# pixeli99/SVD_Xtend

Measured on NVIDIA H100. Metric: SVD UNet train-step frames/sec @ 14x320x512 bf16, higher is better.
Workload: dtype bf16

## Files before the change

### svd_xtend_b200/csrc/tapgemm.cu

```cuda
#include "tapgemm_common.cuh"

namespace svdx {

template <int BN, int TA, int TB>
__device__ __forceinline__ void tile_mainloop(int kb0, int kb1, uint32_t sA, uint32_t sB, uint32_t bar_full, uint32_t bar_empty,
                                           uint32_t sAcc, int wg, int& stage, uint32_t& phase) {
  float acc[BN / 2];
#pragma unroll
  for (int i = 0; i < BN / 2; ++i) acc[i] = 0.f;
  const int lane = threadIdx.x & 31;
  const uint32_t astep = TA ? (2048 >> 4) : (32 >> 4), bstep = TB ? (2048 >> 4) : (32 >> 4);
  int prev_stage = -1;
  for (int kb = kb0; kb < kb1; ++kb) {
    mbar_wait_mma(bar_full + 8 * stage, phase);
    const uint32_t aaddr = sA + stage * A_STAGE_BYTES + wg * 8192;
    const uint32_t baddr = sB + stage * B_STAGE_BYTES;
    const uint64_t ad0 = make_smem_desc_sw128(aaddr, 8192, 1024);
    const uint64_t bd0 = make_smem_desc_sw128(baddr, 8192, 1024);
    wgmma_fence();
#pragma unroll
    for (int j = 0; j < BLOCK_K / 16; ++j) {
      const uint32_t accumulate = (kb > kb0 || j > 0) ? 1u : 0u;
      if constexpr (BN == 32) wgmma_ss_n32<TA, TB>(acc, ad0 + j * astep, bd0 + j * bstep, accumulate);
      else if constexpr (BN == 64) wgmma_ss_n64<TA, TB>(acc, ad0 + j * astep, bd0 + j * bstep, accumulate);
      else if constexpr (BN == 96) wgmma_ss_n96<TA, TB>(acc, ad0 + j * astep, bd0 + j * bstep, accumulate);
      else if constexpr (BN == 128) wgmma_ss_n128<TA, TB>(acc, ad0 + j * astep, bd0 + j * bstep, accumulate);
      else wgmma_ss_n160<TA, TB>(acc, ad0 + j * astep, bd0 + j * bstep, accumulate);
    }
    wgmma_commit();
    wgmma_wait<1>();
    reg_fence(acc);
    if (prev_stage >= 0) {
      __syncwarp();
      if (lane == 0) mbar_arrive(bar_empty + 8 * prev_stage);
    }
    prev_stage = stage;
    if (++stage == STAGES) { stage = 0; phase ^= 1; }
  }
  wgmma_wait<0>();
  reg_fence(acc);
  __syncwarp();
  if (lane == 0 && prev_stage >= 0) mbar_arrive(bar_empty + 8 * prev_stage);

  const int r0 = wg * 64 + ((threadIdx.x >> 5) & 3) * 16 + (lane >> 2);
  const uint32_t base = sAcc + (uint32_t)(r0 * ACC_LD + 2 * (lane & 3)) * 4u;
#pragma unroll
  for (int j = 0; j < BN / 8; ++j) {
#pragma unroll
    for (int h = 0; h < 2; ++h)
      asm volatile("st.shared.v2.f32 [%0], {%1, %2};" ::"r"(base + (uint32_t)(h * 8 * ACC_LD + 8 * j) * 4u), "f"(acc[4 * j + 2 * h]),
                   "f"(acc[4 * j + 2 * h + 1]) : "memory");
  }
}

template <int TA, int TB>
SVDX_DEVINL void tile_mainloop_bn(int bn, int kb0, int kb1, uint32_t sA, uint32_t sB, uint32_t bar_full, uint32_t bar_empty, uint32_t sAcc,
                                  int wg, int& stage, uint32_t& phase) {
  switch (bn) {
    case 32: tile_mainloop<32, TA, TB>(kb0, kb1, sA, sB, bar_full, bar_empty, sAcc, wg, stage, phase); break;
    case 64: tile_mainloop<64, TA, TB>(kb0, kb1, sA, sB, bar_full, bar_empty, sAcc, wg, stage, phase); break;
    case 96: tile_mainloop<96, TA, TB>(kb0, kb1, sA, sB, bar_full, bar_empty, sAcc, wg, stage, phase); break;
    case 128: tile_mainloop<128, TA, TB>(kb0, kb1, sA, sB, bar_full, bar_empty, sAcc, wg, stage, phase); break;
    default: tile_mainloop<160, TA, TB>(kb0, kb1, sA, sB, bar_full, bar_empty, sAcc, wg, stage, phase); break;
  }
}

template <int EPI>
__global__ void __launch_bounds__(NUM_THREADS, 1) tapgemm_kernel(const __grid_constant__ TapGemmKParams p) {
  extern __shared__ uint8_t smem_raw[];
  const uint32_t smem_base = (smem_u32(smem_raw) + 1023u) & ~1023u;
  const uint32_t sA = smem_base;
  const uint32_t sB = smem_base + STAGES * A_STAGE_BYTES;
  const uint32_t sAcc = sB + STAGES * B_STAGE_BYTES;
  const uint32_t sEpi = sAcc + ACC_BYTES;
  const uint32_t sBar = sEpi + NUM_EPI_WARPS * EPI_STAGE_BYTES;
  const uint32_t bar_full = sBar;
  const uint32_t bar_empty = sBar + 8 * STAGES;

  const int warp = threadIdx.x >> 5;
  const int lane = threadIdx.x & 31;

  if (warp == PRODUCER_WARP && lane == 0) {
    prefetch_tmap(&p.tma);
    prefetch_tmap(&p.tmb);
    for (int i = 0; i < STAGES; ++i) {
      mbar_init(bar_full + 8 * i, 1);
      mbar_init(bar_empty + 8 * i, NUM_EPI_WARPS);
    }
    fence_barrier_init();
  }
  __syncthreads();

  const int total_tiles = p.m_tiles * p.n_tiles * p.split_k;
  const int b_bytes = p.block_n * BLOCK_K * 2;

  if (warp == PRODUCER_WARP) {
    const bool conv_par = (p.a_mode == SVDX_A_CONV2D) && !p.a_mn && !p.b_mn && !p.geglu && !p.wtiles && !p.im2col && (BLOCK_M / p.W) <= 32;
    if (conv_par) {
      int stage = 0;
      uint32_t phase = 0;
      for (int tile = blockIdx.x; tile < total_tiles; tile += gridDim.x) {
        const int nt = tile % p.n_tiles;
        const int mt = (tile / p.n_tiles) % p.m_tiles;
        const int ks = tile / (p.n_tiles * p.m_tiles);
        const int kb0 = ks * p.kb_per_split;
        const int kb1 = min(kb0 + p.kb_per_split, p.kb_total);
        const int n0 = nt * p.block_n;
        ConvBox bx;
        conv_tile_boxes(p, mt, lane, bx);
        const CUtensorMap* amap = bx.lg == 0 ? &p.tma : &p.tma_bh[bx.lg - 1];
        int tap = kb0 / p.kb_per_tap;
        int kci = kb0 - tap * p.kb_per_tap;
        for (int kb = kb0; kb < kb1; ++kb) {
          const uint32_t full = bar_full + 8 * stage;
          if (lane == 0) {
            mbar_wait_mma(bar_empty + 8 * stage, phase ^ 1);
            mbar_expect_tx(full, A_STAGE_BYTES + b_bytes);
          }
          __syncwarp();
          const int kc = kci * BLOCK_K;
          if (bx.active)
            tma_load_4d(amap, full, sA + stage * A_STAGE_BYTES + bx.dst_off, kc, p.tap_d0[tap], bx.hh + p.tap_d1[tap],
                        bx.nvalid ? bx.n + p.tap_d2[tap] : (1 << 28));
          if (lane == 0) tma_load_2d(&p.tmb, full, sB + stage * B_STAGE_BYTES, tap * p.K + kc, n0);
          if (++kci == p.kb_per_tap) { kci = 0; ++tap; }
          if (++stage == STAGES) { stage = 0; phase ^= 1; }
        }
      }
    } else if (p.a_mn && p.b_mn && p.b_mode != 1) {
      int stage = 0;
      uint32_t phase = 0;
      const int nb = p.block_n / 64;
      for (int tile = blockIdx.x; tile < total_tiles; tile += gridDim.x) {
        const int nt = tile % p.n_tiles;
        const int mt = (tile / p.n_tiles) % p.m_tiles;
        const int ks = tile / (p.n_tiles * p.m_tiles);
        const int kb0 = ks * p.kb_per_split;
        const int kb1 = min(kb0 + p.kb_per_split, p.kb_total);
        const int n0 = nt * p.block_n;
        int g = 0, kbi = kb0;
        if (p.b_mode == 2) { g = kb0 / p.kb_per_group; kbi = kb0 - g * p.kb_per_group; }
        const int shift = p.b_mode == 2 ? p.tap_d0[0] : 0;
        for (int kb = kb0; kb < kb1; ++kb) {
          const uint32_t full = bar_full + 8 * stage;
          if (lane == 0) {
            mbar_wait_mma(bar_empty + 8 * stage, phase ^ 1);
            mbar_expect_tx(full, A_STAGE_BYTES + b_bytes);
          }
          __syncwarp();
          const uint32_t dA = sA + stage * A_STAGE_BYTES;
          const uint32_t dB = sB + stage * B_STAGE_BYTES;
          if (p.b_mode == 2) {
            const int k0 = kbi * BLOCK_K;
            if (lane < 2) tma_load_3d(&p.tma, full, dA + lane * 8192, mt * BLOCK_M + 64 * lane, k0, g);
            else if (lane < 2 + nb) tma_load_3d(&p.tmb, full, dB + (lane - 2) * 8192, n0 + 64 * (lane - 2), k0 + shift, g);
            if (++kbi == p.kb_per_group) { kbi = 0; ++g; }
          } else {
            if (lane < 2) tma_load_2d(&p.tma, full, dA + lane * 8192, mt * BLOCK_M + 64 * lane, kb * BLOCK_K);
            else if (lane < 2 + nb) tma_load_2d(&p.tmb, full, dB + (lane - 2) * 8192, n0 + 64 * (lane - 2), kb * BLOCK_K);
          }
          if (++stage == STAGES) { stage = 0; phase ^= 1; }
        }
      }
    } else if (lane == 0) {
      int stage = 0;
      uint32_t phase = 0;
      for (int tile = blockIdx.x; tile < total_tiles; tile += gridDim.x) {
        const int nt = tile % p.n_tiles;
        const int mt = (tile / p.n_tiles) % p.m_tiles;
        const int ks = tile / (p.n_tiles * p.m_tiles);
        const int kb0 = ks * p.kb_per_split;
        const int kb1 = min(kb0 + p.kb_per_split, p.kb_total);
        const int n0 = nt * (p.geglu ? p.block_n / 2 : p.block_n);
        int iw = 0, ih = 0, in = 0;
        if (p.im2col && p.a_mode == SVDX_A_CONV2D) {
          const int row = mt * BLOCK_M / p.W;
          iw = mt * BLOCK_M - row * p.W;
          in = row / p.H;
          ih = row - in * p.H;
        }
        int tap = kb0 / p.kb_per_tap;
        int kci = kb0 - tap * p.kb_per_tap - 1;
        for (int kb = kb0; kb < kb1; ++kb) {
          if (++kci == p.kb_per_tap) { kci = 0; ++tap; }
          mbar_wait_mma(bar_empty + 8 * stage, phase ^ 1);
          const uint32_t full = bar_full + 8 * stage;
          mbar_expect_tx(full, A_STAGE_BYTES + b_bytes);
          const uint32_t dA = sA + stage * A_STAGE_BYTES;
          const uint32_t dB = sB + stage * B_STAGE_BYTES;
          const int kc = kci * BLOCK_K;
          if (p.a_mn) {
            if (p.b_mode == 2) {
              const int g = kb / p.kb_per_group;
              const int k0 = (kb - g * p.kb_per_group) * BLOCK_K;
              tma_load_3d(&p.tma, full, dA, mt * BLOCK_M, k0, g);
              tma_load_3d(&p.tma, full, dA + 8192, mt * BLOCK_M + 64, k0, g);
            } else {
              tma_load_2d(&p.tma, full, dA, mt * BLOCK_M, kb * BLOCK_K);
              tma_load_2d(&p.tma, full, dA + 8192, mt * BLOCK_M + 64, kb * BLOCK_K);
            }
          } else if (p.a_mode == SVDX_A_ROWS) {
            const int g = mt / p.tiles_per_group;
            const int t = mt - g * p.tiles_per_group;
            tma_load_3d(&p.tma, full, dA, kc, t * BLOCK_M + p.tap_d0[tap], g);
          } else if (p.im2col) {
            tma_load_4d_im2col(&p.tma, full, dA, kc, iw - 1, ih - 1, in + p.tap_d2[tap], (uint16_t)(p.tap_d0[tap] + 1),
                               (uint16_t)(p.tap_d1[tap] + 1));
          } else if (p.wtiles) {
            const int row = mt / p.wtiles;
            const int w0 = (mt - row * p.wtiles) * BLOCK_M;
            const int n = row / p.H;
            const int h = row - n * p.H;
            tma_load_4d(&p.tma, full, dA, kc, w0 + p.tap_d0[tap], h + p.tap_d1[tap], (n < p.nimg) ? n + p.tap_d2[tap] : (1 << 28));
          } else {
            const int R = BLOCK_M / p.W;
            const int dw = p.tap_d0[tap], dh = p.tap_d1[tap], dn = p.tap_d2[tap];
            int rowid = mt * R, left = R;
            uint32_t dst = dA;
            while (left > 0) {
              const int n = rowid / p.H;
              const int h = rowid - n * p.H;
              const int nn = (n < p.nimg) ? n + dn : (1 << 28);
              int run = min(left, p.H - h);
              int hh = h;
              while (run > 0) {
                int lg = min(p.max_bh_log2, 31 - __clz(run));
                const int bh = 1 << lg;
                tma_load_4d(lg == 0 ? &p.tma : &p.tma_bh[lg - 1], full, dst, kc, dw, hh + dh, nn);
                dst += bh * p.W * 128;
                hh += bh; run -= bh; left -= bh; rowid += bh;
              }
            }
          }
          if (p.b_mn && p.b_mode == 1 && p.im2col) {
            const int pix0 = kb * BLOCK_K;
            const int row = pix0 / p.W;
            const int n = row / p.H;
            for (int j = 0; j < p.block_n / 64; ++j)
              tma_load_4d_im2col(&p.tmb, full, dB + j * 8192, n0 + 64 * j, pix0 - row * p.W - 1, row - n * p.H - 1, n + p.tap_d2[0],
                                 (uint16_t)(p.tap_d0[0] + 1), (uint16_t)(p.tap_d1[0] + 1));
          } else if (p.b_mn && p.b_mode == 1) {
            const int dw = p.tap_d0[0], dh = p.tap_d1[0], dn = p.tap_d2[0];
            const int pix0 = kb * BLOCK_K;
            for (int j = 0; j < p.block_n / 64; ++j) {
              if (p.W >= 64) {
                const int row = pix0 / p.W;
                const int n = row / p.H;
                const int nn = (n < p.nimg) ? n + dn : (1 << 28);
                tma_load_4d(&p.tmb, full, dB + j * 8192, n0 + 64 * j, pix0 - row * p.W + dw, row - n * p.H + dh, nn);
              } else {
                const int R = 64 / p.W;
                for (int i = 0; i < R; ++i) {
                  const int row = pix0 / p.W + i;
                  const int n = row / p.H;
                  const int nn = (n < p.nimg) ? n + dn : (1 << 28);
                  tma_load_4d(&p.tmb, full, dB + j * 8192 + i * p.W * 128, n0 + 64 * j, dw, row - n * p.H + dh, nn);
                }
              }
            }
          } else if (p.b_mn && p.b_mode == 2) {
            const int g = kb / p.kb_per_group;
            const int k0 = (kb - g * p.kb_per_group) * BLOCK_K;
            for (int j = 0; j < p.block_n / 64; ++j)
              tma_load_3d(&p.tmb, full, dB + j * 8192, n0 + 64 * j, k0 + p.tap_d0[0], g);
          } else if (p.b_mn) {
            for (int j = 0; j < p.block_n / 64; ++j)
              tma_load_2d(&p.tmb, full, dB + j * 8192, n0 + 64 * j, kb * BLOCK_K);
          } else if (p.geglu) {
            const int h = p.block_n / 2;
            tma_load_2d(&p.tmb, full, dB, tap * p.K + kc, n0);
            tma_load_2d(&p.tmb, full, dB + h * 128, tap * p.K + kc, p.N / 2 + n0);
          } else {
            tma_load_2d(&p.tmb, full, dB, tap * p.K + kc, n0);
          }
          if (++stage == STAGES) { stage = 0; phase ^= 1; }
        }
      }
    }
  } else {
    const int wg = warp >> 2;
    const int q = warp & 3;
    const int half = warp >> 2;
    int stage = 0;
    uint32_t phase = 0;
    float s_acc = 1.f, s_r1 = 1.f, s_r2 = 1.f;
    if (p.scales) { s_acc = p.scales[0]; s_r1 = p.scales[1]; s_r2 = p.scales[2]; }
    const int n_out_total = p.geglu ? p.N / 2 : p.N;
    const int bn_out = p.geglu ? p.block_n / 2 : p.block_n;
    EpiStage st;
    st.base = sEpi + warp * EPI_STAGE_BYTES;
    st.off = 0;
    const uint32_t t_base = sAcc + (uint32_t)((q * 32 + lane) * ACC_LD) * 4u;
    for (int tile = blockIdx.x; tile < total_tiles; tile += gridDim.x) {
      const int nt = tile % p.n_tiles;
      const int mt = (tile / p.n_tiles) % p.m_tiles;
      const int ks = tile / (p.n_tiles * p.m_tiles);
      const int kb0 = ks * p.kb_per_split;
      const int kb1 = min(kb0 + p.kb_per_split, p.kb_total);
      const int n0 = nt * bn_out;
      long long m;
      bool row_ok;
      tile_row(p, mt, q * 32 + lane, m, row_ok);
      if (p.a_mode == SVDX_A_ROWS && !p.a_mn) {
        st.grp = mt / p.tiles_per_group;
        st.row0 = (mt - st.grp * p.tiles_per_group) * BLOCK_M + q * 32;
      } else {
        st.grp = 0;
        st.row0 = mt * BLOCK_M + q * 32;
      }
      long long m0;
      int valid_rows;
      if (p.a_mode == SVDX_A_ROWS && !p.a_mn) {
        m0 = (long long)st.grp * p.rows_per_group + st.row0;
        valid_rows = max(0, min(32, p.rows_per_group - st.row0));
      } else {
        m0 = st.row0;
        valid_rows = max(0, min(32, p.M - st.row0));
      }
      if constexpr (EPI == EPI_RES || EPI == EPI_RES_GN || EPI == EPI_FAST_GNB)
        prefetch_epilogue_operands(p, EPI, m0, valid_rows, n0, bn_out, n_out_total, lane, half);
      named_bar_sync(1, 32 * NUM_EPI_WARPS);
      if (p.a_mn && p.b_mn) tile_mainloop_bn<1, 1>(p.block_n, kb0, kb1, sA, sB, bar_full, bar_empty, sAcc, wg, stage, phase);
      else if (p.a_mn) tile_mainloop_bn<1, 0>(p.block_n, kb0, kb1, sA, sB, bar_full, bar_empty, sAcc, wg, stage, phase);
      else if (p.b_mn) tile_mainloop_bn<0, 1>(p.block_n, kb0, kb1, sA, sB, bar_full, bar_empty, sAcc, wg, stage, phase);
      else tile_mainloop_bn<0, 0>(p.block_n, kb0, kb1, sA, sB, bar_full, bar_empty, sAcc, wg, stage, phase);
      named_bar_sync(1, 32 * NUM_EPI_WARPS);
      if constexpr (EPI == EPI_FAST || EPI == EPI_FAST_GN) epilogue_fast<EPI == EPI_FAST_GN>(p, t_base, m, row_ok, n0, half, 0, bn_out, n_out_total, st.base, st.row0, st.grp, lane, m0, valid_rows);
      else if constexpr (EPI == EPI_FAST_IL || EPI == EPI_FAST_IL_GN) epilogue_fast<EPI == EPI_FAST_IL_GN, true>(p, t_base, m, row_ok, n0, half, 0, bn_out, n_out_total, st.base, st.row0, st.grp, lane, m0, valid_rows);
      else if constexpr (EPI == EPI_FAST_ACT) epilogue_fast<false, false, true>(p, t_base, m, row_ok, n0, half, 0, bn_out, n_out_total, st.base, st.row0, st.grp, lane, m0, valid_rows);
      else if constexpr (EPI == EPI_RES || EPI == EPI_RES_GN) epilogue_res<EPI == EPI_RES_GN>(p, t_base, m, row_ok, n0, half, 0, bn_out, n_out_total, s_acc, s_r1, s_r2, st.base, st.off, st.row0, st.grp, lane, m0, valid_rows);
      else if constexpr (EPI == EPI_GEGLU) epilogue_geglu(p, t_base, n0, half, bn_out, st.base, st.row0, st.grp, lane);
      else if constexpr (EPI == EPI_FAST_GNB) epilogue_fast_gnb(p, t_base, m, row_ok, n0, half, 0, bn_out, n_out_total, st.base, st.row0, st.grp, lane, m0, valid_rows);
      else epilogue_tile(p, t_base, m, row_ok, n0, half, bn_out, n_out_total, s_acc, s_r1, s_r2, st, lane);
    }
    if (lane == 0) bulk_wait<0>();
  }
}

}

using namespace svdx;

static int kernel_block_n(int block_n, bool step64) {
  const int step = step64 ? 64 : 32, cap = step64 ? 128 : MAX_BN;
  if (block_n <= cap) return block_n;
  for (int w = cap; w > step; w -= step)
    if (block_n % w == 0) return w;
  return step;
}

int svdx_tapgemm_fill(const SvdxTapGemm* d, TapGemmKParams& p) {
  if (!d || !d->a || !d->b || !d->out) return svdx_fail(SVDX_E_BADARG, "tapgemm: null pointer");
  const bool wide320 = d->block_n == 320;
  if (wide320 && (d->geglu || d->N % 320 || d->M < 512 || d->out_dtype != SVDX_OUT_BF16))
    return svdx_fail(SVDX_E_BADARG, "tapgemm: block_n 320 needs N %% 320 == 0, M >= 512 and a bf16 output without GEGLU");
  if (!wide320 && (d->block_n < 32 || d->block_n > 256 || d->block_n % 32))
    return svdx_fail(SVDX_E_BADARG, "tapgemm: block_n must be a multiple of 32 in [32,256] (or 320)");
  if (d->b_major_mn && d->block_n % 64) return svdx_fail(SVDX_E_BADARG, "tapgemm: block_n %% 64 for MN-major B");
  if (d->num_taps < 1 || d->num_taps > SVDX_MAX_TAPS) return svdx_fail(SVDX_E_BADARG, "tapgemm: num_taps");
  if (d->M <= 0 || d->N <= 0 || d->K <= 0) return svdx_fail(SVDX_E_BADARG, "tapgemm: empty problem");
  if (d->split_k < 1 || (d->split_k > 1 && d->out_dtype != SVDX_OUT_F32_ATOMIC)) return svdx_fail(SVDX_E_BADARG, "tapgemm: split_k needs atomic output");
  if (d->geglu && (d->N % 2 || d->block_n % 64 || d->b_major_mn || (d->N / 2) % (d->block_n / 2))) return svdx_fail(SVDX_E_BADARG, "tapgemm: geglu shape");
  if ((d->lda % 8) || (d->ldb % 8)) return svdx_fail(SVDX_E_BADARG, "tapgemm: lda/ldb must be multiples of 8 elements (16 B)");
  if ((reinterpret_cast<uintptr_t>(d->a) & 15) || (reinterpret_cast<uintptr_t>(d->b) & 15)) return svdx_fail(SVDX_E_BADARG, "tapgemm: operands must be 16 B aligned");
  if ((d->a_major_mn || d->b_major_mn) && (d->a_mode != SVDX_A_ROWS || d->num_taps != 1)) return svdx_fail(SVDX_E_BADARG, "tapgemm: MN-major operands only in single-tap ROWS mode");
  if (d->b_mode != 0 && !(d->a_major_mn && d->b_major_mn)) return svdx_fail(SVDX_E_BADARG, "tapgemm: b_mode needs MN-major A and B (weight-gradient form)");

  memset(&p, 0, sizeof(p));
  p.a_mode = d->a_mode; p.a_mn = d->a_major_mn; p.b_mn = d->b_major_mn;
  p.num_taps = d->num_taps;
  for (int i = 0; i < d->num_taps; ++i) { p.tap_d0[i] = d->tap_d0[i]; p.tap_d1[i] = d->tap_d1[i]; p.tap_d2[i] = d->tap_d2[i]; }
  const int block_n = kernel_block_n(d->block_n, d->b_major_mn || d->geglu);
  p.M = d->M; p.N = d->N; p.K = d->K; p.block_n = block_n; p.split_k = d->split_k;
  p.geglu = d->geglu;
  const int bn_out = d->geglu ? block_n / 2 : block_n;
  const int n_out = d->geglu ? d->N / 2 : d->N;
  p.n_tiles = (n_out + bn_out - 1) / bn_out;

  int rc;
  p.b_mode = d->b_mode;
  if (d->a_major_mn) {
    if (d->groups > 1 && d->b_mode != 2) return svdx_fail(SVDX_E_BADARG, "tapgemm: MN-major A requires groups==1");
    if (d->b_mode == 2) {
      uint64_t dims[3] = {(uint64_t)d->M, (uint64_t)d->rows_per_group, (uint64_t)d->groups};
      uint64_t strides[2] = {(uint64_t)d->lda * 2, (uint64_t)d->lda * 2 * (uint64_t)d->rows_per_group};
      uint32_t box[3] = {64, 64, 1};
      rc = svdx_make_tmap(&p.tma, d->a, 3, dims, strides, box);
    } else {
      uint64_t dims[2] = {(uint64_t)d->M, (uint64_t)d->K};
      uint64_t strides[1] = {(uint64_t)d->lda * 2};
      uint32_t box[2] = {64, 64};
      rc = svdx_make_tmap(&p.tma, d->a, 2, dims, strides, box);
    }
    p.rows_per_group = d->M; p.groups = 1; p.tiles_per_group = (d->M + BLOCK_M - 1) / BLOCK_M;
    p.m_tiles = p.tiles_per_group;
  } else if (d->a_mode == SVDX_A_ROWS) {
    if (d->rows_per_group <= 0 || d->groups <= 0 || (long long)d->rows_per_group * d->groups != d->M) return svdx_fail(SVDX_E_BADARG, "tapgemm: rows_per_group*groups != M");
    uint64_t dims[3] = {(uint64_t)d->K, (uint64_t)d->rows_per_group, (uint64_t)d->groups};
    uint64_t strides[2] = {(uint64_t)d->lda * 2, (uint64_t)d->lda * 2 * (uint64_t)d->rows_per_group};
    uint32_t box[3] = {64, 128, 1};
    rc = svdx_make_tmap(&p.tma, d->a, 3, dims, strides, box);
    p.rows_per_group = d->rows_per_group; p.groups = d->groups;
    p.tiles_per_group = (d->rows_per_group + BLOCK_M - 1) / BLOCK_M;
    p.m_tiles = p.tiles_per_group * d->groups;
  } else if (d->a_mode == SVDX_A_CONV2D) {
    const bool wide = d->W > 128;
    if (d->W <= 0 || d->H <= 0 || d->nimg <= 0) return svdx_fail(SVDX_E_BADARG, "tapgemm: conv2d needs W, H, images > 0");
    const bool boxes = wide ? (d->W % 128 == 0) : (128 % d->W == 0);
    uint64_t dims[4] = {(uint64_t)d->K, (uint64_t)d->W, (uint64_t)d->H, (uint64_t)d->nimg};
    uint64_t strides[3] = {(uint64_t)d->lda * 2, (uint64_t)d->lda * 2 * d->W, (uint64_t)d->lda * 2 * d->W * d->H};
    uint32_t box[4] = {64, (uint32_t)(wide ? 128 : d->W), 1, 1};
    p.max_bh_log2 = 0;
    if (!boxes) {
      for (int i = 0; i < d->num_taps; ++i)
        if (d->tap_d0[i] < -1 || d->tap_d0[i] > 1 || d->tap_d1[i] < -1 || d->tap_d1[i] > 1)
          return svdx_fail(SVDX_E_BADARG, "tapgemm: conv2d at a width with neither W | 128 nor 128 | W needs taps with |dw|, |dh| <= 1");
      rc = svdx_make_tmap_im2col(&p.tma, d->a, dims, strides, BLOCK_M);
      p.im2col = 1;
    } else {
      rc = svdx_make_tmap(&p.tma, d->a, 4, dims, strides, box);
    }
    p.wtiles = (wide && boxes) ? d->W / 128 : 0;
    for (int lg = 1; lg <= 4 && !rc && !wide && boxes; ++lg) {
      const int bh = 1 << lg;
      if (bh * d->W > BLOCK_M || bh > d->H) break;
      uint32_t boxh[4] = {64, (uint32_t)d->W, (uint32_t)bh, 1};
      rc = svdx_make_tmap(&p.tma_bh[lg - 1], d->a, 4, dims, strides, boxh);
      p.max_bh_log2 = lg;
    }
    p.W = d->W; p.H = d->H; p.nimg = d->M / (d->H * d->W);
    if ((long long)p.nimg * d->H * d->W != d->M) return svdx_fail(SVDX_E_BADARG, "tapgemm: conv2d M must be images*H*W");
    p.m_tiles = (d->M + BLOCK_M - 1) / BLOCK_M;
    p.rows_per_group = d->M; p.groups = 1; p.tiles_per_group = p.m_tiles;
  } else {
    return svdx_fail(SVDX_E_BADARG, "tapgemm: a_mode");
  }
  if (rc) return rc;

  if (d->b_major_mn && d->b_mode == 1) {
    if (d->W <= 0 || d->H <= 0 || d->nimg <= 0) return svdx_fail(SVDX_E_BADARG, "tapgemm: b_mode 1 needs W, H, images > 0");
    uint64_t dims[4] = {(uint64_t)d->N, (uint64_t)d->W, (uint64_t)d->H, (uint64_t)d->nimg};
    uint64_t strides[3] = {(uint64_t)d->ldb * 2, (uint64_t)d->ldb * 2 * d->W, (uint64_t)d->ldb * 2 * d->W * d->H};
    uint32_t box[4] = {64, (uint32_t)(d->W >= 64 ? 64 : d->W), 1, 1};
    if ((d->W < 64 && 64 % d->W) || (d->W >= 64 && d->W % 64)) {
      if (d->tap_d0[0] < -1 || d->tap_d0[0] > 1 || d->tap_d1[0] < -1 || d->tap_d1[0] > 1)
        return svdx_fail(SVDX_E_BADARG, "tapgemm: b_mode 1 at a width with neither W | 64 nor 64 | W needs a tap with |dw|, |dh| <= 1");
      rc = svdx_make_tmap_im2col(&p.tmb, d->b, dims, strides, 64);
      p.im2col = 1;
    } else {
      rc = svdx_make_tmap(&p.tmb, d->b, 4, dims, strides, box);
    }
    p.W = d->W; p.H = d->H; p.nimg = d->K / (d->W * d->H);
    if ((long long)p.nimg * d->W * d->H != d->K) return svdx_fail(SVDX_E_BADARG, "tapgemm: b_mode 1 K must be images*H*W");
  } else if (d->b_major_mn && d->b_mode == 2) {
    if (d->rows_per_group <= 0 || d->groups <= 0 || (long long)d->rows_per_group * d->groups != d->K) return svdx_fail(SVDX_E_BADARG, "tapgemm: b_mode 2 rows_per_group*groups != K");
    uint64_t dims[3] = {(uint64_t)d->N, (uint64_t)d->rows_per_group, (uint64_t)d->groups};
    uint64_t strides[2] = {(uint64_t)d->ldb * 2, (uint64_t)d->ldb * 2 * (uint64_t)d->rows_per_group};
    uint32_t box[3] = {64, 64, 1};
    rc = svdx_make_tmap(&p.tmb, d->b, 3, dims, strides, box);
    p.rows_per_group = d->rows_per_group; p.groups = d->groups;
  } else if (d->b_major_mn) {
    uint64_t dims[2] = {(uint64_t)d->N, (uint64_t)d->K};
    uint64_t strides[1] = {(uint64_t)d->ldb * 2};
    uint32_t box[2] = {64, 64};
    rc = svdx_make_tmap(&p.tmb, d->b, 2, dims, strides, box);
  } else {
    uint64_t dims[2] = {(uint64_t)d->K * d->num_taps, (uint64_t)d->N};
    uint64_t strides[1] = {(uint64_t)d->ldb * 2};
    uint32_t box[2] = {64, (uint32_t)(d->geglu ? block_n / 2 : block_n)};
    rc = svdx_make_tmap(&p.tmb, d->b, 2, dims, strides, box);
  }
  if (rc) return rc;

  p.kb_per_tap = (d->K + BLOCK_K - 1) / BLOCK_K;
  p.kb_total = p.kb_per_tap * d->num_taps;
  p.kb_per_group = p.kb_per_tap;
  if (d->b_mode == 2) {
    p.kb_per_group = (d->rows_per_group + BLOCK_K - 1) / BLOCK_K;
    p.kb_per_tap = p.kb_per_group * d->groups;
    p.kb_total = p.kb_per_tap;
  }
  p.kb_per_split = (p.kb_total + d->split_k - 1) / d->split_k;
  p.split_k = (p.kb_total + p.kb_per_split - 1) / p.kb_per_split;

  p.out = d->out; p.ldo = d->ldo; p.out_dtype = d->out_dtype;
  p.bias = d->bias; p.rowbias = d->rowbias; p.rowbias_div = d->rowbias_div > 0 ? d->rowbias_div : 1; p.ldrb = d->ldrb;
  p.res1 = reinterpret_cast<const bf16*>(d->res1); p.ldr1 = d->ldr1;
  p.res2 = reinterpret_cast<const bf16*>(d->res2); p.ldr2 = d->ldr2;
  p.scales = d->scales; p.pre = reinterpret_cast<bf16*>(d->pre); p.ldpre = d->ldpre;
  p.gn_sum = d->gn_sum; p.gn_ld = d->gn_ld; p.gn_rows = d->gn_rows;
  p.gnb_x = reinterpret_cast<const bf16*>(d->gnb_x); p.gnb_ldx = d->gnb_ldx; p.gnb_c1 = d->gnb_x2 ? d->gnb_c1 : d->N;
  p.gnb_x2 = reinterpret_cast<const bf16*>(d->gnb_x2); p.gnb_ldx2 = d->gnb_ldx2;
  p.gnb_ab = d->gnb_ab; p.gnb_sum = d->gnb_sum; p.gnb_rows = d->gnb_rows; p.gnb_silu = d->gnb_silu;
  {
    static int probe = -1;
    if (probe < 0) { const char* e = getenv("SVDX_EPI_PROBE"); probe = e ? atoi(e) : 0; }
    p.probe = probe;
  }
  {
    static int use = -1;
    if (use < 0) { const char* e = getenv("SVDX_TMA_STORE"); use = e ? atoi(e) : 1; }
    const bool grouped = (d->a_mode == SVDX_A_ROWS && !d->a_major_mn);
    const uint64_t R = grouped ? (uint64_t)d->rows_per_group : (uint64_t)d->M;
    const uint64_t G = grouped ? (uint64_t)d->groups : 1;
    const bool f32 = d->out_dtype != SVDX_OUT_BF16;
    const int esz = f32 ? 4 : 2;
    bool ok = use != 0 && (d->ldo * esz) % 16 == 0 && (reinterpret_cast<uintptr_t>(d->out) & 15) == 0;
    if (d->geglu && d->pre && ((d->N / 2) % 32 || (d->ldpre % 8) || (reinterpret_cast<uintptr_t>(d->pre) & 15))) ok = false;
    if (ok) {
      uint64_t dims[3] = {(uint64_t)n_out, R, G};
      uint64_t strides[2] = {(uint64_t)d->ldo * esz, (uint64_t)d->ldo * esz * R};
      uint32_t box[3] = {32, 32, 1};
      rc = svdx_make_tmap_ex(&p.tmo, d->out, f32, f32 ? 128 : 64, 3, dims, strides, box);
      if (rc) return rc;
      if (d->geglu && d->pre) {
        uint64_t pdims[3] = {(uint64_t)d->N, R, G};
        uint64_t pstrides[2] = {(uint64_t)d->ldpre * 2, (uint64_t)d->ldpre * 2 * R};
        rc = svdx_make_tmap_ex(&p.tmpre, d->pre, 0, 64, 3, pdims, pstrides, box);
        if (rc) return rc;
      }
      p.tma_store = 1;
    }
    p.epi_mode = EPI_GENERIC;
    const bool vec_ok = (reinterpret_cast<uintptr_t>(d->bias) & 15) == 0
                        && (!d->rowbias || ((reinterpret_cast<uintptr_t>(d->rowbias) & 15) == 0 && d->ldrb % 4 == 0));
    if (p.tma_store && !f32 && n_out % 32 == 0 && vec_ok && !p.probe && use != 2)
      p.epi_mode = d->geglu ? EPI_GEGLU : (d->res1 || d->res2 || d->scales) ? EPI_RES : EPI_FAST;
  }
  if (p.split_k > 1 && (p.bias || p.rowbias || p.res1 || p.res2 || p.geglu)) return svdx_fail(SVDX_E_BADARG, "tapgemm: split_k with epilogue operands");
  if (p.gnb_sum) {
    if (p.epi_mode != EPI_FAST || p.gn_sum)
      return svdx_fail(SVDX_E_BADARG, "tapgemm: gnb_sum needs the plain bf16 TMA-store epilogue (no residual / scales / GEGLU / split-K / gn_sum)");
    if (!p.gnb_x || p.gnb_rows <= 0 || (p.gnb_silu && !p.gnb_ab) || (d->N & 1) || (p.gnb_ldx % 8) || (reinterpret_cast<uintptr_t>(p.gnb_x) & 15) ||
        (reinterpret_cast<uintptr_t>(p.gnb_sum) & 7) || (p.gnb_ab && (reinterpret_cast<uintptr_t>(p.gnb_ab) & 7)) ||
        (p.gnb_x2 && (p.gnb_c1 <= 0 || p.gnb_c1 >= d->N || p.gnb_c1 % 32 || (p.gnb_ldx2 % 8) || (reinterpret_cast<uintptr_t>(p.gnb_x2) & 15))))
      return svdx_fail(SVDX_E_BADARG, "tapgemm: gnb operands (x rows 16-byte aligned, gnb_rows > 0, scale/shift table for SiLU, concat split % 32)");
    p.epi_mode = EPI_FAST_GNB;
  }
  if (d->interleave) {
    if (d->a_mode != SVDX_A_CONV2D || d->a_major_mn || d->b_major_mn || (d->phase_h & ~1) || (d->phase_w & ~1))
      return svdx_fail(SVDX_E_BADARG, "tapgemm: interleave needs CONV2D mode and phases in {0, 1}");
    if (p.epi_mode != EPI_FAST || p.rowbias || p.split_k > 1 || p.gnb_sum)
      return svdx_fail(SVDX_E_BADARG, "tapgemm: interleave needs the plain bf16 TMA-store epilogue (bias only: no rowbias / residual / "
                                      "scales / GEGLU / split-K / gnb sums; N %% 32 == 0, aligned rows)");
    if (p.W < 32 && 32 % p.W)
      return svdx_fail(SVDX_E_BADARG, "tapgemm: interleave with W < 32 needs W | 32 (a store chunk is whole image rows)");
    if (p.W < 32 && (p.H * p.W) % 32)
      return svdx_fail(SVDX_E_BADARG, "tapgemm: interleave with W < 32 needs H*W %% 32 == 0 (a store chunk must not straddle images)");
    const uint64_t rb = (uint64_t)d->ldo * 2;
    uint64_t dims[4] = {(uint64_t)n_out, (uint64_t)p.W, (uint64_t)p.H, (uint64_t)p.nimg};
    uint64_t strides[3] = {2 * rb, 4 * (uint64_t)p.W * rb, 4 * (uint64_t)p.W * p.H * rb};
    uint32_t box[4] = {32, (uint32_t)(p.W < 32 ? p.W : 32), (uint32_t)(p.W < 32 ? 32 / p.W : 1), 1};
    const bf16* base = reinterpret_cast<const bf16*>(d->out) + (2LL * p.W * d->phase_h + d->phase_w) * d->ldo;
    rc = svdx_make_tmap_ex(&p.tmo, base, 0, 64, 4, dims, strides, box);
    if (rc) return rc;
    p.il_out = const_cast<bf16*>(base);
    p.interleave = 1;
    p.epi_mode = EPI_FAST_IL;
  }
  if (d->act != SVDX_ACT_NONE) {
    if (d->act != SVDX_ACT_GELU && d->act != SVDX_ACT_QUICK_GELU) return svdx_fail(SVDX_E_BADARG, "tapgemm: act must be SVDX_ACT_GELU or SVDX_ACT_QUICK_GELU");
    if (p.epi_mode != EPI_FAST || p.rowbias || p.split_k > 1 || p.gn_sum)
      return svdx_fail(SVDX_E_BADARG, "tapgemm: act needs the plain bf16 TMA-store epilogue (bias only: no rowbias / residual / scales / "
                                      "GEGLU / split-K / gn_sum / gnb sums / interleave; N %% 32 == 0, aligned rows)");
    p.act = d->act;
    p.epi_mode = EPI_FAST_ACT;
  }
  if (wide320 && p.epi_mode != EPI_FAST && p.epi_mode != EPI_RES && p.epi_mode != EPI_FAST_GNB && p.epi_mode != EPI_FAST_IL && p.epi_mode != EPI_FAST_ACT)
    return svdx_fail(SVDX_E_BADARG, "tapgemm: block_n 320 needs a bf16 output through the TMA-store epilogues (N % 320 == 0, aligned rows)");
  if (p.gn_sum) {
    if (p.epi_mode != EPI_FAST && p.epi_mode != EPI_RES && p.epi_mode != EPI_FAST_IL)
      return svdx_fail(SVDX_E_BADARG, "tapgemm: gn_sum needs a bf16 output through the TMA-store epilogues (N % 32 == 0, aligned rows), no split-K / GEGLU");
    if (p.gn_rows <= 0 || p.gn_ld < n_out || (p.gn_ld & 1) || (reinterpret_cast<uintptr_t>(p.gn_sum) & 7))
      return svdx_fail(SVDX_E_BADARG, "tapgemm: gn_sum needs gn_rows > 0, even gn_ld >= N, 8-byte aligned buffer");
  }
  if (d->out_dtype == SVDX_OUT_BF16 && ((d->ldo % 8) || (reinterpret_cast<uintptr_t>(d->out) & 15))) return svdx_fail(SVDX_E_BADARG, "tapgemm: out alignment");
  if (d->out_dtype != SVDX_OUT_BF16 && ((d->ldo % 4) || (reinterpret_cast<uintptr_t>(d->out) & 15))) return svdx_fail(SVDX_E_BADARG, "tapgemm: out alignment");
  if (d->res1 && ((d->ldr1 % 8) || (reinterpret_cast<uintptr_t>(d->res1) & 15))) return svdx_fail(SVDX_E_BADARG, "tapgemm: res1 alignment");
  if (d->res2 && ((d->ldr2 % 8) || (reinterpret_cast<uintptr_t>(d->res2) & 15))) return svdx_fail(SVDX_E_BADARG, "tapgemm: res2 alignment");
  if (d->pre && ((d->ldpre % 8) || (reinterpret_cast<uintptr_t>(d->pre) & 15))) return svdx_fail(SVDX_E_BADARG, "tapgemm: pre alignment");

  return SVDX_OK;
}

extern "C" int svdx_tapgemm(const SvdxTapGemm* d, void* stream_v) {
  cudaStream_t stream = reinterpret_cast<cudaStream_t>(stream_v);
  TapGemmKParams p;
  int rc = svdx_tapgemm_fill(d, p);
  if (rc) return rc;
  static bool attr_done[SVDX_MAX_DEVICES] = {false};
  const int slot = svdx_device_slot();
  if (!attr_done[slot]) {
    cudaError_t e = cudaFuncSetAttribute(tapgemm_kernel<EPI_GENERIC>, cudaFuncAttributeMaxDynamicSharedMemorySize, SMEM_BYTES);
    if (e == cudaSuccess) e = cudaFuncSetAttribute(tapgemm_kernel<EPI_FAST>, cudaFuncAttributeMaxDynamicSharedMemorySize, SMEM_BYTES);
    if (e == cudaSuccess) e = cudaFuncSetAttribute(tapgemm_kernel<EPI_GEGLU>, cudaFuncAttributeMaxDynamicSharedMemorySize, SMEM_BYTES);
    if (e == cudaSuccess) e = cudaFuncSetAttribute(tapgemm_kernel<EPI_RES>, cudaFuncAttributeMaxDynamicSharedMemorySize, SMEM_BYTES);
    if (e == cudaSuccess) e = cudaFuncSetAttribute(tapgemm_kernel<EPI_FAST_GN>, cudaFuncAttributeMaxDynamicSharedMemorySize, SMEM_BYTES);
    if (e == cudaSuccess) e = cudaFuncSetAttribute(tapgemm_kernel<EPI_RES_GN>, cudaFuncAttributeMaxDynamicSharedMemorySize, SMEM_BYTES);
    if (e == cudaSuccess) e = cudaFuncSetAttribute(tapgemm_kernel<EPI_FAST_GNB>, cudaFuncAttributeMaxDynamicSharedMemorySize, SMEM_BYTES);
    if (e == cudaSuccess) e = cudaFuncSetAttribute(tapgemm_kernel<EPI_FAST_IL>, cudaFuncAttributeMaxDynamicSharedMemorySize, SMEM_BYTES);
    if (e == cudaSuccess) e = cudaFuncSetAttribute(tapgemm_kernel<EPI_FAST_IL_GN>, cudaFuncAttributeMaxDynamicSharedMemorySize, SMEM_BYTES);
    if (e == cudaSuccess) e = cudaFuncSetAttribute(tapgemm_kernel<EPI_FAST_ACT>, cudaFuncAttributeMaxDynamicSharedMemorySize, SMEM_BYTES);
    if (e != cudaSuccess) return svdx_fail_cuda(e, "tapgemm: set smem attribute");
    attr_done[slot] = true;
  }
  const int total_tiles = p.m_tiles * p.n_tiles * p.split_k;
  int grid = svdx_num_sms();
  if (grid > total_tiles) grid = total_tiles;
  if (p.epi_mode == EPI_FAST_ACT) tapgemm_kernel<EPI_FAST_ACT><<<grid, NUM_THREADS, SMEM_BYTES, stream>>>(p);
  else if (p.epi_mode == EPI_FAST_IL && p.gn_sum) tapgemm_kernel<EPI_FAST_IL_GN><<<grid, NUM_THREADS, SMEM_BYTES, stream>>>(p);
  else if (p.epi_mode == EPI_FAST_IL) tapgemm_kernel<EPI_FAST_IL><<<grid, NUM_THREADS, SMEM_BYTES, stream>>>(p);
  else if (p.epi_mode == EPI_FAST_GNB) tapgemm_kernel<EPI_FAST_GNB><<<grid, NUM_THREADS, SMEM_BYTES, stream>>>(p);
  else if (p.epi_mode == EPI_FAST && p.gn_sum) tapgemm_kernel<EPI_FAST_GN><<<grid, NUM_THREADS, SMEM_BYTES, stream>>>(p);
  else if (p.epi_mode == EPI_RES && p.gn_sum) tapgemm_kernel<EPI_RES_GN><<<grid, NUM_THREADS, SMEM_BYTES, stream>>>(p);
  else if (p.epi_mode == EPI_FAST) tapgemm_kernel<EPI_FAST><<<grid, NUM_THREADS, SMEM_BYTES, stream>>>(p);
  else if (p.epi_mode == EPI_GEGLU) tapgemm_kernel<EPI_GEGLU><<<grid, NUM_THREADS, SMEM_BYTES, stream>>>(p);
  else if (p.epi_mode == EPI_RES) tapgemm_kernel<EPI_RES><<<grid, NUM_THREADS, SMEM_BYTES, stream>>>(p);
  else tapgemm_kernel<EPI_GENERIC><<<grid, NUM_THREADS, SMEM_BYTES, stream>>>(p);
  cudaError_t e = cudaGetLastError();
  if (e != cudaSuccess) return svdx_fail_cuda(e, "tapgemm: launch");
  return SVDX_OK;
}
```

### svd_xtend_b200/csrc/tapgemm_common.cuh

```cuda
#pragma once
#include "common.cuh"
#include "../../include/svd_xtend_b200.h"
#include "host_util.h"

namespace svdx {

constexpr int BLOCK_M = 128;
constexpr int BLOCK_K = 64;
constexpr int STAGES = 3;
constexpr int MAX_BN = 160;
constexpr int A_STAGE_BYTES = BLOCK_M * BLOCK_K * 2;
constexpr int B_STAGE_BYTES = MAX_BN * BLOCK_K * 2;
constexpr int NUM_EPI_WARPS = 8;
constexpr int PRODUCER_WARP = NUM_EPI_WARPS;
constexpr int NUM_THREADS = 32 * NUM_EPI_WARPS + 32;
constexpr int ACC_LD = MAX_BN + 4;
constexpr int ACC_BYTES = BLOCK_M * ACC_LD * 4;
constexpr int EPI_STAGE_BYTES = 4096;
constexpr int SMEM_BYTES = 1024 + STAGES * (A_STAGE_BYTES + B_STAGE_BYTES) + ACC_BYTES + NUM_EPI_WARPS * EPI_STAGE_BYTES + 256;
static_assert(SMEM_BYTES <= 227 * 1024, "tapgemm shared memory exceeds the 227 KB a block may use");
static_assert((ACC_BYTES % 1024) == 0 && (B_STAGE_BYTES % 1024) == 0, "staging buffers must stay 1024-byte aligned");

struct __align__(64) TapGemmKParams {
  CUtensorMap tma;
  CUtensorMap tmb;
  CUtensorMap tma_bh[4];
  int max_bh_log2;
  int a_mode, a_mn, b_mn, b_mode, kb_per_group;
  int rows_per_group, groups, tiles_per_group;
  int W, H, nimg;
  int wtiles;
  int im2col;
  int num_taps;
  int tap_d0[SVDX_MAX_TAPS], tap_d1[SVDX_MAX_TAPS], tap_d2[SVDX_MAX_TAPS];
  int M, N, K;
  int block_n, m_tiles, n_tiles, split_k, kb_total, kb_per_split, kb_per_tap;
  void* out;
  long long ldo;
  int out_dtype, geglu;
  const float* bias;
  const float* rowbias;
  int rowbias_div;
  long long ldrb;
  const bf16* res1;
  long long ldr1;
  const bf16* res2;
  long long ldr2;
  const float* scales;
  bf16* pre;
  long long ldpre;
  CUtensorMap tmo;
  CUtensorMap tmpre;
  float* gn_sum;
  long long gn_ld;
  int gn_rows;
  const bf16* gnb_x;
  long long gnb_ldx;
  const bf16* gnb_x2;
  long long gnb_ldx2;
  int gnb_c1;
  const float* gnb_ab;
  float* gnb_sum;
  int gnb_rows, gnb_silu;
  int tma_store;
  int epi_mode;
  int probe;
  int interleave;
  int act;
  bf16* il_out;
};


SVDX_DEVINL void acc_ld32(uint32_t row, int col, uint32_t (&r)[32]) {
  const uint32_t a = row + col * 4;
#pragma unroll
  for (int k = 0; k < 8; ++k)
    asm volatile("ld.shared.v4.b32 {%0, %1, %2, %3}, [%4];" : "=r"(r[4 * k]), "=r"(r[4 * k + 1]), "=r"(r[4 * k + 2]), "=r"(r[4 * k + 3])
                 : "r"(a + 16 * k));
}

SVDX_DEVINL void tile_row(const TapGemmKParams& p, int mt, int r, long long& m, bool& row_ok) {
  if (p.a_mode == SVDX_A_ROWS && !p.a_mn) {
    const int g = mt / p.tiles_per_group;
    const int t = mt - g * p.tiles_per_group;
    const int rin = t * BLOCK_M + r;
    row_ok = rin < p.rows_per_group;
    m = (long long)g * p.rows_per_group + rin;
  } else {
    m = (long long)mt * BLOCK_M + r;
    row_ok = m < p.M;
  }
}

struct ConvBox {
  int lg, hh, n;
  uint32_t dst_off;
  bool nvalid, active;
};
SVDX_DEVINL void conv_tile_boxes(const TapGemmKParams& p, int t, int lane, ConvBox& mine) {
  const int R = BLOCK_M / p.W;
  int rowid = t * R, left = R, idx = 0;
  uint32_t off = 0;
  mine.active = false; mine.lg = 0; mine.hh = 0; mine.n = 0; mine.dst_off = 0; mine.nvalid = false;
  while (left > 0) {
    const int n = rowid / p.H;
    const int h = rowid - n * p.H;
    int run = min(left, p.H - h);
    int hh = h;
    while (run > 0) {
      const int lg = min(p.max_bh_log2, 31 - __clz(run));
      const int bh = 1 << lg;
      if (idx == lane) { mine.lg = lg; mine.hh = hh; mine.n = n; mine.nvalid = n < p.nimg; mine.dst_off = off; mine.active = true; }
      off += bh * p.W * 128;
      hh += bh; run -= bh; left -= bh; rowid += bh; ++idx;
    }
  }
}

struct EpiStage {
  uint32_t base;
  uint32_t off;
  int row0, grp;
};

SVDX_DEVINL void stage_store_bf16(const CUtensorMap* tm, EpiStage& st, int lane, const float (&f)[32], int col) {
  if (lane == 0) bulk_wait_read<1>();
  __syncwarp();
  const uint32_t buf = st.base + st.off;
  const uint32_t row = buf + lane * 64;
  const int sw = (lane >> 1) & 3;
#pragma unroll
  for (int j = 0; j < 4; ++j)
    st_shared_v4(row + ((j ^ sw) << 4), pack_bf16x2(f[8 * j], f[8 * j + 1]), pack_bf16x2(f[8 * j + 2], f[8 * j + 3]),
                 pack_bf16x2(f[8 * j + 4], f[8 * j + 5]), pack_bf16x2(f[8 * j + 6], f[8 * j + 7]));
  fence_proxy_async_smem();
  __syncwarp();
  if (lane == 0) { tma_store_3d(tm, buf, col, st.row0, st.grp); bulk_commit(); }
  st.off ^= 2048;
}

SVDX_DEVINL void stage_store_f32(const CUtensorMap* tm, EpiStage& st, int lane, const float (&f)[32], int col, bool reduce) {
  if (lane == 0) bulk_wait_read<0>();
  __syncwarp();
  const uint32_t row = st.base + lane * 128;
  const int sw = lane & 7;
#pragma unroll
  for (int j = 0; j < 8; ++j)
    st_shared_v4(row + ((j ^ sw) << 4), __float_as_uint(f[4 * j]), __float_as_uint(f[4 * j + 1]), __float_as_uint(f[4 * j + 2]),
                 __float_as_uint(f[4 * j + 3]));
  fence_proxy_async_smem();
  __syncwarp();
  if (lane == 0) {
    if (reduce) tma_reduce_add_3d(tm, st.base, col, st.row0, st.grp);
    else tma_store_3d(tm, st.base, col, st.row0, st.grp);
    bulk_commit();
  }
}

SVDX_DEVINL void gn_chunk_sums(const TapGemmKParams& p, uint32_t buf, int lane, int col0, int n_out_total, long long m0, int valid_rows) {
  const int pr = lane & 15, h = lane >> 4;
  const uint32_t in_chunk = (uint32_t)(pr & 3) * 4u;
  const int jch = pr >> 2;
  long long slab = m0 / p.gn_rows;
  int left = p.gn_rows - (int)(m0 - slab * p.gn_rows);
  int r = 0;
  while (r < valid_rows) {
    const int seg_end = min(valid_rows, r + left);
    float s0 = 0.f, s1 = 0.f, q0 = 0.f, q1 = 0.f;
    for (int rr = r + ((h ^ r) & 1); rr < seg_end; rr += 2) {
      uint32_t w;
      asm volatile("ld.shared.u32 %0, [%1];" : "=r"(w) : "r"(buf + rr * 64 + ((uint32_t)(jch ^ ((rr >> 1) & 3)) << 4) + in_chunk));
      const float2 v = unpack_bf16x2(w);
      s0 += v.x; s1 += v.y;
      q0 = fmaf(v.x, v.x, q0); q1 = fmaf(v.y, v.y, q1);
    }
    s0 += __shfl_xor_sync(0xffffffffu, s0, 16); s1 += __shfl_xor_sync(0xffffffffu, s1, 16);
    q0 += __shfl_xor_sync(0xffffffffu, q0, 16); q1 += __shfl_xor_sync(0xffffffffu, q1, 16);
    const int col = col0 + 2 * pr;
    if (h == 0 && col < n_out_total) {
      float* d = p.gn_sum + (2 * slab) * p.gn_ld + col;
      asm volatile("red.global.add.v2.f32 [%0], {%1, %2};" ::"l"(d), "f"(s0), "f"(s1) : "memory");
      asm volatile("red.global.add.v2.f32 [%0], {%1, %2};" ::"l"(d + p.gn_ld), "f"(q0), "f"(q1) : "memory");
    }
    r = seg_end; ++slab; left = p.gn_rows;
  }
}

constexpr int EPI_GENERIC = 0, EPI_FAST = 1, EPI_GEGLU = 2, EPI_RES = 3;
constexpr int EPI_FAST_GN = 4, EPI_RES_GN = 5;
constexpr int EPI_FAST_GNB = 6;
constexpr int EPI_FAST_IL = 7, EPI_FAST_IL_GN = 8;
constexpr int EPI_FAST_ACT = 9;

SVDX_DEVINL void act32(float (&f)[32], int act) {
  if (act == SVDX_ACT_GELU) {
#pragma unroll
    for (int i = 0; i < 32; ++i) f[i] = gelu_erf_f(f[i]);
  } else {
#pragma unroll
    for (int i = 0; i < 32; ++i) f[i] = __fdividef(f[i], 1.0f + __expf(-1.702f * f[i]));
  }
}

template <bool IL>
SVDX_DEVINL void store_chunk(const TapGemmKParams& p, uint32_t src, int col, int row0, int grp) {
  if constexpr (IL) {
    const int w0 = row0 % p.W, r = row0 / p.W;
    tma_store_4d(&p.tmo, src, col, w0, r % p.H, r / p.H);
  } else {
    tma_store_3d(&p.tmo, src, col, row0, grp);
  }
}

SVDX_DEVINL void il_store_next_row(const TapGemmKParams& p, uint32_t src, int col, int row0, int lane) {
  const int k = p.W - row0 % p.W;
  if (p.W < 32 || k >= 32 || lane < k || row0 + lane >= p.M) return;
  const long long orow = 4LL * p.W * (row0 / p.W + 1) + 2 * (lane - k);
  uint4* dst = reinterpret_cast<uint4*>(p.il_out + orow * p.ldo + col);
  const uint32_t row = src + lane * 64;
  const int sw = (lane >> 1) & 3;
#pragma unroll
  for (int j = 0; j < 4; ++j) {
    uint4 v;
    asm volatile("ld.shared.v4.b32 {%0, %1, %2, %3}, [%4];" : "=r"(v.x), "=r"(v.y), "=r"(v.z), "=r"(v.w) : "r"(row + ((j ^ sw) << 4)));
    dst[j] = v;
  }
}

SVDX_DEVINL void add_vec32(float (&f)[32], const float* __restrict__ src) {
  const float4* bp = reinterpret_cast<const float4*>(src);
#pragma unroll
  for (int k = 0; k < 8; ++k) {
    const float4 b4 = __ldg(bp + k);
    f[4 * k] += b4.x; f[4 * k + 1] += b4.y; f[4 * k + 2] += b4.z; f[4 * k + 3] += b4.w;
  }
}
SVDX_DEVINL void axpy_bf16x32(float (&f)[32], float s, const uint4 (&r)[4]) {
#pragma unroll
  for (int k = 0; k < 4; ++k) {
    const float2 a = unpack_bf16x2(r[k].x), b = unpack_bf16x2(r[k].y), c = unpack_bf16x2(r[k].z), d = unpack_bf16x2(r[k].w);
    f[8 * k] += s * a.x; f[8 * k + 1] += s * a.y; f[8 * k + 2] += s * b.x; f[8 * k + 3] += s * b.y;
    f[8 * k + 4] += s * c.x; f[8 * k + 5] += s * c.y; f[8 * k + 6] += s * d.x; f[8 * k + 7] += s * d.y;
  }
}
SVDX_DEVINL void stage_row_bf16(uint32_t row, int sw, const float (&f)[32]) {
#pragma unroll
  for (int j = 0; j < 4; ++j)
    st_shared_v4(row + ((j ^ sw) << 4), pack_bf16x2(f[8 * j], f[8 * j + 1]), pack_bf16x2(f[8 * j + 2], f[8 * j + 3]),
                 pack_bf16x2(f[8 * j + 4], f[8 * j + 5]), pack_bf16x2(f[8 * j + 6], f[8 * j + 7]));
}

SVDX_DEVINL void prefetch_rows_l2(const bf16* base, long long ld, long long m0, int valid_rows, int col0, int ncols, int lane, int half) {
  if (!base || lane >= valid_rows) return;
  const char* row = reinterpret_cast<const char*>(base + (m0 + lane) * ld + col0);
  const int bytes = ncols * 2;
  for (int b = half * 128; b < bytes; b += 256) asm volatile("prefetch.global.L2 [%0];" ::"l"(row + b));
}
SVDX_DEVINL void prefetch_epilogue_operands(const TapGemmKParams& p, int epi, long long m0, int valid_rows, int n0, int bn_out, int n_out_total,
                                            int lane, int half) {
  const int ncols = min(bn_out, n_out_total - n0);
  if (ncols <= 0) return;
  if (epi == EPI_RES || epi == EPI_RES_GN) {
    prefetch_rows_l2(p.res1, p.ldr1, m0, valid_rows, n0, ncols, lane, half);
    prefetch_rows_l2(p.res2, p.ldr2, m0, valid_rows, n0, ncols, lane, half);
  } else if (epi == EPI_FAST_GNB) {
    if (n0 < p.gnb_c1) prefetch_rows_l2(p.gnb_x, p.gnb_ldx, m0, valid_rows, n0, min(ncols, p.gnb_c1 - n0), lane, half);
    if (n0 + ncols > p.gnb_c1) {
      const int c0 = max(n0, p.gnb_c1);
      prefetch_rows_l2(p.gnb_x2, p.gnb_ldx2, m0, valid_rows, c0 - p.gnb_c1, n0 + ncols - c0, lane, half);
    }
  }
}

template <bool GN, bool IL = false, bool ACT = false>
SVDX_DEVINL void epilogue_fast(const TapGemmKParams& p, uint32_t t_base, long long m, bool row_ok, int n0, int half, int c_lo, int c_hi,
                               int n_out_total, uint32_t sbase, int row0, int grp, int lane, long long m0, int valid_rows) {
  const float* bias = p.bias;
  const float* rb = (p.rowbias && row_ok) ? p.rowbias + (m / p.rowbias_div) * p.ldrb : nullptr;
  const uint32_t rowX = sbase + lane * 64, rowY = rowX + 2048;
  const int sw = (lane >> 1) & 3;
#pragma unroll 1
  for (int c = c_lo + half * 32; c < c_hi; c += 128) {
    const int colA = n0 + c;
    if (colA >= n_out_total) break;
    const int colB = colA + 64;
    const bool hasB = (c + 64 < c_hi) && (colB < n_out_total);
    uint32_t va[32], vb[32];
    acc_ld32(t_base, c, va);
    if (hasB) acc_ld32(t_base, c + 64, vb);
    float fa[32], fb[32];
#pragma unroll
    for (int i = 0; i < 32; ++i) { fa[i] = __uint_as_float(va[i]); fb[i] = __uint_as_float(vb[i]); }
    if (bias) { add_vec32(fa, bias + colA); if (hasB) add_vec32(fb, bias + colB); }
    if (rb) { add_vec32(fa, rb + colA); if (hasB) add_vec32(fb, rb + colB); }
    if constexpr (ACT) { act32(fa, p.act); if (hasB) act32(fb, p.act); }
    if (lane == 0) bulk_wait_read<0>();
    __syncwarp();
    stage_row_bf16(rowX, sw, fa);
    if (hasB) stage_row_bf16(rowY, sw, fb);
    fence_proxy_async_smem();
    __syncwarp();
    if (lane == 0) {
      store_chunk<IL>(p, sbase, colA, row0, grp);
      if (hasB) store_chunk<IL>(p, sbase + 2048, colB, row0, grp);
      bulk_commit();
    }
    if constexpr (IL) {
      il_store_next_row(p, sbase, colA, row0, lane);
      if (hasB) il_store_next_row(p, sbase + 2048, colB, row0, lane);
    }
    if constexpr (GN) {
      gn_chunk_sums(p, sbase, lane, colA, n_out_total, m0, valid_rows);
      if (hasB) gn_chunk_sums(p, sbase + 2048, lane, colB, n_out_total, m0, valid_rows);
    }
  }
}

SVDX_DEVINL void gnb_chunk_sums(const TapGemmKParams& p, uint32_t buf_dy, uint32_t buf_x, int lane, int col0, int n_out_total, long long m0,
                                int valid_rows) {
  const int pr = lane & 15, h = lane >> 4;
  const uint32_t in_chunk = (uint32_t)(pr & 3) * 4u;
  const int jch = pr >> 2;
  long long slab = m0 / p.gnb_rows;
  int left = p.gnb_rows - (int)(m0 - slab * p.gnb_rows);
  const int col = col0 + 2 * pr;
  const bool col_ok = col < n_out_total;
  int r = 0;
  while (r < valid_rows) {
    const int seg_end = min(valid_rows, r + left);
    float2 A = make_float2(0.f, 0.f), B = make_float2(0.f, 0.f);
    if (col_ok && p.gnb_silu) {
      A = *reinterpret_cast<const float2*>(p.gnb_ab + (2 * slab) * p.N + col);
      B = *reinterpret_cast<const float2*>(p.gnb_ab + (2 * slab + 1) * p.N + col);
    }
    float s0 = 0.f, s1 = 0.f, x0 = 0.f, x1 = 0.f;
    if (r == 0 && seg_end == 32) {
#pragma unroll
      for (int b = 0; b < 2; ++b) {
        uint32_t wd[8], wx[8];
#pragma unroll
        for (int i = 0; i < 8; ++i) {
          const int rr = h + 2 * (8 * b + i);
          const uint32_t off = rr * 64 + ((uint32_t)(jch ^ ((rr >> 1) & 3)) << 4) + in_chunk;
          asm volatile("ld.shared.u32 %0, [%1];" : "=r"(wd[i]) : "r"(buf_dy + off));
          asm volatile("ld.shared.u32 %0, [%1];" : "=r"(wx[i]) : "r"(buf_x + off));
        }
        float e0[8], e1[8];
#pragma unroll
        for (int i = 0; i < 8; ++i) {
          const float2 d = unpack_bf16x2(wd[i]), xv = unpack_bf16x2(wx[i]);
          e0[i] = d.x; e1[i] = d.y;
          if (p.gnb_silu) {
            e0[i] *= silu_grad_f(fmaf(xv.x, A.x, B.x));
            e1[i] *= silu_grad_f(fmaf(xv.y, A.y, B.y));
          }
        }
#pragma unroll
        for (int i = 0; i < 8; ++i) {
          const float2 xv = unpack_bf16x2(wx[i]);
          s0 += e0[i]; s1 += e1[i];
          x0 = fmaf(e0[i], xv.x, x0); x1 = fmaf(e1[i], xv.y, x1);
        }
      }
    } else {
      for (int rr = r + ((h ^ r) & 1); rr < seg_end; rr += 2) {
        const uint32_t off = rr * 64 + ((uint32_t)(jch ^ ((rr >> 1) & 3)) << 4) + in_chunk;
        uint32_t wd, wx;
        asm volatile("ld.shared.u32 %0, [%1];" : "=r"(wd) : "r"(buf_dy + off));
        asm volatile("ld.shared.u32 %0, [%1];" : "=r"(wx) : "r"(buf_x + off));
        const float2 d = unpack_bf16x2(wd), xv = unpack_bf16x2(wx);
        float e0 = d.x, e1 = d.y;
        if (p.gnb_silu) {
          e0 *= silu_grad_f(fmaf(xv.x, A.x, B.x));
          e1 *= silu_grad_f(fmaf(xv.y, A.y, B.y));
        }
        s0 += e0; s1 += e1;
        x0 = fmaf(e0, xv.x, x0); x1 = fmaf(e1, xv.y, x1);
      }
    }
    s0 += __shfl_xor_sync(0xffffffffu, s0, 16); s1 += __shfl_xor_sync(0xffffffffu, s1, 16);
    x0 += __shfl_xor_sync(0xffffffffu, x0, 16); x1 += __shfl_xor_sync(0xffffffffu, x1, 16);
    if (h == 0 && col_ok) {
      float* d = p.gnb_sum + (2 * slab) * p.N + col;
      asm volatile("red.global.add.v2.f32 [%0], {%1, %2};" ::"l"(d), "f"(s0), "f"(s1) : "memory");
      asm volatile("red.global.add.v2.f32 [%0], {%1, %2};" ::"l"(d + p.N), "f"(x0), "f"(x1) : "memory");
    }
    r = seg_end; ++slab; left = p.gnb_rows;
  }
}

SVDX_DEVINL void epilogue_fast_gnb(const TapGemmKParams& p, uint32_t t_base, long long m, bool row_ok, int n0, int half, int c_lo, int c_hi,
                                   int n_out_total, uint32_t sbase, int row0, int grp, int lane, long long m0, int valid_rows) {
  const float* bias = p.bias;
  const float* rb = (p.rowbias && row_ok) ? p.rowbias + (m / p.rowbias_div) * p.ldrb : nullptr;
  const uint32_t rowX = sbase + lane * 64;
  const int sw = (lane >> 1) & 3;
  const int prow = lane >> 2, ppc = lane & 3;
#pragma unroll 1
  for (int c = c_lo + half * 32; c < c_hi; c += 64) {
    const int col0 = n0 + c;
    if (col0 >= n_out_total) break;
    const bool src1 = col0 < p.gnb_c1;
    const long long xld = src1 ? p.gnb_ldx : p.gnb_ldx2;
    const bf16* xs = (src1 ? p.gnb_x + col0 : p.gnb_x2 + (col0 - p.gnb_c1)) + m0 * xld + ppc * 8;
    uint4 xa[4];
#pragma unroll
    for (int j = 0; j < 4; ++j) {
      const int rr = prow + 8 * j;
      xa[j] = (rr < valid_rows) ? *reinterpret_cast<const uint4*>(xs + (long long)rr * xld) : make_uint4(0u, 0u, 0u, 0u);
    }
    uint32_t v[32];
    acc_ld32(t_base, c, v);
    float f[32];
#pragma unroll
    for (int i = 0; i < 32; ++i) f[i] = __uint_as_float(v[i]);
    if (bias) add_vec32(f, bias + col0);
    if (rb) add_vec32(f, rb + col0);
    if (lane == 0) bulk_wait_read<0>();
    __syncwarp();
    stage_row_bf16(rowX, sw, f);
#pragma unroll
    for (int j = 0; j < 4; ++j) {
      const int rr = prow + 8 * j;
      st_shared_v4(sbase + 2048 + rr * 64 + ((ppc ^ ((rr >> 1) & 3)) << 4), xa[j].x, xa[j].y, xa[j].z, xa[j].w);
    }
    fence_proxy_async_smem();
    __syncwarp();
    if (lane == 0) { tma_store_3d(&p.tmo, sbase, col0, row0, grp); bulk_commit(); }
    gnb_chunk_sums(p, sbase, sbase + 2048, lane, col0, n_out_total, m0, valid_rows);
    __syncwarp();
  }
}

template <bool GN>
SVDX_DEVINL void epilogue_res(const TapGemmKParams& p, uint32_t t_base, long long m, bool row_ok, int n0, int half, int c_lo, int c_hi,
                              int n_out_total, float s_acc, float s_r1, float s_r2, uint32_t sbase, uint32_t& off, int row0, int grp, int lane,
                              long long m0, int valid_rows) {
  const float* bias = p.bias;
  const float* rb = (p.rowbias && row_ok) ? p.rowbias + (m / p.rowbias_div) * p.ldrb : nullptr;
  const bf16* r1 = p.res1 ? p.res1 + m0 * p.ldr1 : nullptr;
  const bf16* r2 = (p.res2 && row_ok) ? p.res2 + m * p.ldr2 : nullptr;
  const bool scaled = p.scales != nullptr;
  const uint32_t row = sbase + lane * 64;
  const int sw = (lane >> 1) & 3;
  const int prow = lane >> 2, ppc = lane & 3;
#pragma unroll 1
  for (int c = c_lo + half * 32; c < c_hi; c += 64) {
    const int col0 = n0 + c;
    if (col0 >= n_out_total) break;
    uint4 a1[4], a2[4];
    if (r1) {
#pragma unroll
      for (int j = 0; j < 4; ++j) {
        const int rr = prow + 8 * j;
        a1[j] = (rr < valid_rows) ? *reinterpret_cast<const uint4*>(r1 + (long long)rr * p.ldr1 + col0 + ppc * 8) : make_uint4(0u, 0u, 0u, 0u);
      }
    }
    if (r2) {
      const uint4* q = reinterpret_cast<const uint4*>(r2 + col0);
#pragma unroll
      for (int k = 0; k < 4; ++k) a2[k] = q[k];
    }
    uint32_t v[32];
    acc_ld32(t_base, c, v);
    float f[32];
#pragma unroll
    for (int i = 0; i < 32; ++i) f[i] = __uint_as_float(v[i]);
    if (bias) add_vec32(f, bias + col0);
    if (rb) add_vec32(f, rb + col0);
    if (scaled) {
#pragma unroll
      for (int i = 0; i < 32; ++i) f[i] *= s_acc;
    }
    if (lane == 0) bulk_wait_read<1>();
    __syncwarp();
    if (r1) {
#pragma unroll
      for (int j = 0; j < 4; ++j) {
        const int rr = prow + 8 * j;
        st_shared_v4(sbase + off + rr * 64 + ((ppc ^ ((rr >> 1) & 3)) << 4), a1[j].x, a1[j].y, a1[j].z, a1[j].w);
      }
      __syncwarp();
#pragma unroll
      for (int k = 0; k < 4; ++k)
        asm volatile("ld.shared.v4.b32 {%0, %1, %2, %3}, [%4];" : "=r"(a1[k].x), "=r"(a1[k].y), "=r"(a1[k].z), "=r"(a1[k].w) : "r"(row + off + ((k ^ sw) << 4)));
      axpy_bf16x32(f, s_r1, a1);
    }
    if (r2) axpy_bf16x32(f, s_r2, a2);
    stage_row_bf16(row + off, sw, f);
    fence_proxy_async_smem();
    __syncwarp();
    if (lane == 0) { tma_store_3d(&p.tmo, sbase + off, col0, row0, grp); bulk_commit(); }
    if constexpr (GN) gn_chunk_sums(p, sbase + off, lane, col0, n_out_total, m0, valid_rows);
    off ^= 2048;
  }
}

SVDX_DEVINL void epilogue_geglu(const TapGemmKParams& p, uint32_t t_base, int n0, int half, int bn_out, uint32_t sbase, int row0,
                                int grp, int lane) {
  const float* bias = p.bias;
  const bool save_pre = p.pre != nullptr;
  const int nh = p.N / 2;
  const uint32_t rowX = sbase + lane * 64, rowY = rowX + 2048;
  const int sw = (lane >> 1) & 3;
  uint32_t off = 0;
#pragma unroll 1
  for (int c = half * 32; c < bn_out; c += 64) {
    const int col0 = n0 + c;
    uint32_t v[32], gte[32];
    acc_ld32(t_base, c, v);
    acc_ld32(t_base, bn_out + c, gte);
    float f[32], g[32];
#pragma unroll
    for (int i = 0; i < 32; ++i) { f[i] = __uint_as_float(v[i]); g[i] = __uint_as_float(gte[i]); }
    if (bias) { add_vec32(f, bias + col0); add_vec32(g, bias + nh + col0); }
    if (save_pre) {
      if (lane == 0) bulk_wait_read<0>();
      __syncwarp();
      stage_row_bf16(rowX, sw, f);
      stage_row_bf16(rowY, sw, g);
      fence_proxy_async_smem();
      __syncwarp();
      if (lane == 0) {
        tma_store_3d(&p.tmpre, sbase, col0, row0, grp);
        tma_store_3d(&p.tmpre, sbase + 2048, nh + col0, row0, grp);
        bulk_commit();
      }
    }
#pragma unroll
    for (int i = 0; i < 32; ++i) {
      const float fv = __bfloat162float(__float2bfloat16(f[i]));
      const float gv = __bfloat162float(__float2bfloat16(g[i]));
      f[i] = fv * gelu_erf_f(gv);
    }
    if (save_pre) {
      if (lane == 0) bulk_wait_read<0>();
    } else {
      if (lane == 0) bulk_wait_read<1>();
    }
    __syncwarp();
    stage_row_bf16(save_pre ? rowX : rowX + off, sw, f);
    fence_proxy_async_smem();
    __syncwarp();
    if (lane == 0) { tma_store_3d(&p.tmo, save_pre ? sbase : sbase + off, col0, row0, grp); bulk_commit(); }
    off ^= 2048;
  }
}

SVDX_DEVINL void epilogue_tile(const TapGemmKParams& p, uint32_t t_base, long long m, bool row_ok, int n0, int half, int bn_out,
                               int n_out_total, float s_acc, float s_r1, float s_r2, EpiStage& st, int lane) {
      if (p.probe == 2) return;
      const float* rb = (p.rowbias && row_ok) ? p.rowbias + (m / p.rowbias_div) * p.ldrb : nullptr;
      for (int c = half * 32; c < bn_out; c += 64) {
        uint32_t v[32];
        uint32_t gte[32];
        const int col0 = n0 + c;
        if (col0 >= n_out_total) break;
        const bool full_chunk = (col0 + 32 <= n_out_total);
        uint4 rr1[4], rr2[4];
        if (row_ok && full_chunk) {
          if (p.res1) {
            const uint4* r1p = reinterpret_cast<const uint4*>(p.res1 + m * p.ldr1 + col0);
#pragma unroll
            for (int k = 0; k < 4; ++k) rr1[k] = r1p[k];
          }
          if (p.res2) {
            const uint4* r2p = reinterpret_cast<const uint4*>(p.res2 + m * p.ldr2 + col0);
#pragma unroll
            for (int k = 0; k < 4; ++k) rr2[k] = r2p[k];
          }
        }
        __syncwarp();
        acc_ld32(t_base, c, v);
        if (p.geglu) acc_ld32(t_base, bn_out + c, gte);
        float f[32];
#pragma unroll
        for (int i = 0; i < 32; ++i) f[i] = __uint_as_float(v[i]);
        if (p.geglu) {
          float g[32];
#pragma unroll
          for (int i = 0; i < 32; ++i) g[i] = __uint_as_float(gte[i]);
          if (p.bias) {
            if (full_chunk && ((p.N / 2) & 3) == 0) {
              const float4* bv = reinterpret_cast<const float4*>(p.bias + col0);
              const float4* bg = reinterpret_cast<const float4*>(p.bias + p.N / 2 + col0);
#pragma unroll
              for (int k = 0; k < 8; ++k) {
                const float4 x4 = __ldg(bv + k), y4 = __ldg(bg + k);
                f[4 * k] += x4.x; f[4 * k + 1] += x4.y; f[4 * k + 2] += x4.z; f[4 * k + 3] += x4.w;
                g[4 * k] += y4.x; g[4 * k + 1] += y4.y; g[4 * k + 2] += y4.z; g[4 * k + 3] += y4.w;
              }
            } else {
#pragma unroll
              for (int i = 0; i < 32; ++i) {
                if (full_chunk || col0 + i < n_out_total) {
                  f[i] += __ldg(p.bias + col0 + i);
                  g[i] += __ldg(p.bias + p.N / 2 + col0 + i);
                }
              }
            }
          }
          if (p.pre) {
            if (p.tma_store) {
              stage_store_bf16(&p.tmpre, st, lane, f, col0);
              stage_store_bf16(&p.tmpre, st, lane, g, p.N / 2 + col0);
            } else if (row_ok) {
              bf16* pv = p.pre + m * p.ldpre + col0;
              bf16* pg = pv + p.N / 2;
              if (full_chunk) {
#pragma unroll
                for (int i = 0; i < 32; i += 8) {
                  uint4 a, b;
                  a.x = pack_bf16x2(f[i], f[i + 1]); a.y = pack_bf16x2(f[i + 2], f[i + 3]);
                  a.z = pack_bf16x2(f[i + 4], f[i + 5]); a.w = pack_bf16x2(f[i + 6], f[i + 7]);
                  b.x = pack_bf16x2(g[i], g[i + 1]); b.y = pack_bf16x2(g[i + 2], g[i + 3]);
                  b.z = pack_bf16x2(g[i + 4], g[i + 5]); b.w = pack_bf16x2(g[i + 6], g[i + 7]);
                  *reinterpret_cast<uint4*>(pv + i) = a;
                  *reinterpret_cast<uint4*>(pg + i) = b;
                }
              } else {
                for (int i = 0; i < 32; ++i)
                  if (col0 + i < n_out_total) { pv[i] = __float2bfloat16(f[i]); pg[i] = __float2bfloat16(g[i]); }
              }
            }
          }
#pragma unroll
          for (int i = 0; i < 32; ++i) {
            const float fv = __bfloat162float(__float2bfloat16(f[i]));
            const float gv = __bfloat162float(__float2bfloat16(g[i]));
            f[i] = fv * gelu_erf_f(gv);
          }
        } else {
          if (p.bias) {
            if (full_chunk) {
              const float4* bp = reinterpret_cast<const float4*>(p.bias + col0);
#pragma unroll
              for (int k = 0; k < 8; ++k) {
                const float4 b4 = __ldg(bp + k);
                f[4 * k] += b4.x; f[4 * k + 1] += b4.y; f[4 * k + 2] += b4.z; f[4 * k + 3] += b4.w;
              }
            } else {
              for (int i = 0; i < 32; ++i)
                if (col0 + i < n_out_total) f[i] += __ldg(p.bias + col0 + i);
            }
          }
        }
        if (rb) {
          if (full_chunk && (reinterpret_cast<uintptr_t>(rb + col0) & 15) == 0) {
            const float4* bp = reinterpret_cast<const float4*>(rb + col0);
#pragma unroll
            for (int k = 0; k < 8; ++k) {
              const float4 b4 = __ldg(bp + k);
              f[4 * k] += b4.x; f[4 * k + 1] += b4.y; f[4 * k + 2] += b4.z; f[4 * k + 3] += b4.w;
            }
          } else {
#pragma unroll
            for (int i = 0; i < 32; ++i)
              if (full_chunk || col0 + i < n_out_total) f[i] += __ldg(rb + col0 + i);
          }
        }
        if (p.scales) {
#pragma unroll
          for (int i = 0; i < 32; ++i) f[i] *= s_acc;
        }
        if (p.res1 && row_ok) {
          const bf16* r1 = p.res1 + m * p.ldr1 + col0;
          if (full_chunk) {
#pragma unroll
            for (int i = 0; i < 32; i += 8) {
              const uint4 u = rr1[i >> 3];
              float2 a = unpack_bf16x2(u.x), b = unpack_bf16x2(u.y), c2 = unpack_bf16x2(u.z), d = unpack_bf16x2(u.w);
              f[i] += s_r1 * a.x; f[i + 1] += s_r1 * a.y; f[i + 2] += s_r1 * b.x; f[i + 3] += s_r1 * b.y;
              f[i + 4] += s_r1 * c2.x; f[i + 5] += s_r1 * c2.y; f[i + 6] += s_r1 * d.x; f[i + 7] += s_r1 * d.y;
            }
          } else {
            for (int i = 0; i < 32; ++i)
              if (col0 + i < n_out_total) f[i] += s_r1 * __bfloat162float(r1[i]);
          }
        }
        if (p.res2 && row_ok) {
          const bf16* r2 = p.res2 + m * p.ldr2 + col0;
          if (full_chunk) {
#pragma unroll
            for (int i = 0; i < 32; i += 8) {
              const uint4 u = rr2[i >> 3];
              float2 a = unpack_bf16x2(u.x), b = unpack_bf16x2(u.y), c2 = unpack_bf16x2(u.z), d = unpack_bf16x2(u.w);
              f[i] += s_r2 * a.x; f[i + 1] += s_r2 * a.y; f[i + 2] += s_r2 * b.x; f[i + 3] += s_r2 * b.y;
              f[i + 4] += s_r2 * c2.x; f[i + 5] += s_r2 * c2.y; f[i + 6] += s_r2 * d.x; f[i + 7] += s_r2 * d.y;
            }
          } else {
            for (int i = 0; i < 32; ++i)
              if (col0 + i < n_out_total) f[i] += s_r2 * __bfloat162float(r2[i]);
          }
        }
        if (p.probe == 1) {
          float acc = 0.f;
#pragma unroll
          for (int i = 0; i < 32; ++i) acc += f[i];
          if (acc == 123.456f) reinterpret_cast<float*>(p.out)[0] = acc;
        } else if (p.tma_store) {
          if (p.out_dtype == SVDX_OUT_BF16) stage_store_bf16(&p.tmo, st, lane, f, col0);
          else stage_store_f32(&p.tmo, st, lane, f, col0, p.out_dtype == SVDX_OUT_F32_ATOMIC);
        } else if (!row_ok) {
        } else if (p.out_dtype == SVDX_OUT_BF16) {
          bf16* o = reinterpret_cast<bf16*>(p.out) + m * p.ldo + col0;
          if (full_chunk) {
#pragma unroll
            for (int i = 0; i < 32; i += 8) {
              uint4 a;
              a.x = pack_bf16x2(f[i], f[i + 1]); a.y = pack_bf16x2(f[i + 2], f[i + 3]);
              a.z = pack_bf16x2(f[i + 4], f[i + 5]); a.w = pack_bf16x2(f[i + 6], f[i + 7]);
              *reinterpret_cast<uint4*>(o + i) = a;
            }
          } else {
            for (int i = 0; i < 32; ++i)
              if (col0 + i < n_out_total) o[i] = __float2bfloat16(f[i]);
          }
        } else if (p.out_dtype == SVDX_OUT_F32) {
          float* o = reinterpret_cast<float*>(p.out) + m * p.ldo + col0;
          if (full_chunk) {
#pragma unroll
            for (int i = 0; i < 32; i += 4)
              *reinterpret_cast<float4*>(o + i) = make_float4(f[i], f[i + 1], f[i + 2], f[i + 3]);
          } else {
            for (int i = 0; i < 32; ++i)
              if (col0 + i < n_out_total) o[i] = f[i];
          }
        } else {
          float* o = reinterpret_cast<float*>(p.out) + m * p.ldo + col0;
          if (full_chunk) {
#pragma unroll
            for (int i = 0; i < 32; i += 4)
              asm volatile("red.global.add.v4.f32 [%0], {%1, %2, %3, %4};" ::"l"(o + i), "f"(f[i]), "f"(f[i + 1]), "f"(f[i + 2]), "f"(f[i + 3])
                           : "memory");
          } else {
            for (int i = 0; i < 32; ++i)
              if (col0 + i < n_out_total) atomicAdd(o + i, f[i]);
          }
        }
      }
}

}

int svdx_tapgemm_fill(const SvdxTapGemm* d, svdx::TapGemmKParams& p);
```

### svd_xtend_b200/raw.py

```python
from __future__ import annotations

import ctypes as C
import os
from typing import Optional, Sequence

import torch

from . import _lib
from ._lib import ACT_GELU, ACT_NONE, ACT_QUICK_GELU, A_CONV2D, A_ROWS, OUT_BF16, OUT_F32, OUT_F32_ATOMIC, SvdxAttn, SvdxTapGemm, load

bf16 = torch.bfloat16

_DTYPE_CODE = {torch.float32: 0, torch.bfloat16: 1, torch.float16: 2}


def dtype_code(t: torch.Tensor, what: str) -> int:
    try:
        return _DTYPE_CODE[t.dtype]
    except KeyError:
        raise TypeError(f"svd_xtend_b200: {what} has dtype {t.dtype}; supported: float32, bfloat16, float16") from None

LAUNCHES = [0]
_KERNELS_PER_CALL = {"svdx_groupnorm_apply_fused": 1, "svdx_attention_bwd": 3, "svdx_adamw_graph": 2, "svdx_adamw_p2p": 2,
                     "svdx_adamw_graph_ema": 2, "svdx_adamw_p2p_ema": 2, "svdx_ema_multi": 2, "svdx_adamw8bit": 2,
                     "svdx_adamw8bit_ema": 2}


def check(rc: int, what: str = "") -> None:
    LAUNCHES[0] += _KERNELS_PER_CALL.get(what, 1)
    _lib.check(rc, what)


ABLATE: set = set()
ACCOUNT = None
SHAPE_LOG = None


def _fam(family: str, flops: float = 0.0, nbytes: float = 0.0) -> bool:
    if ACCOUNT is not None:
        ACCOUNT(family, flops, nbytes)
    return family in ABLATE


def _stream() -> int:
    return torch.cuda.current_stream().cuda_stream


def _ptr(t: Optional[torch.Tensor]) -> Optional[int]:
    return None if t is None else t.data_ptr()


def _rowmajor(t: torch.Tensor, name: str) -> int:
    if t.stride(-1) != 1:
        raise ValueError(f"{name}: last dimension must be contiguous")
    return t.stride(-2)


def pick_block_n(n_out: int, mn_major: bool = False) -> int:
    if mn_major:
        for bn in (256, 192, 128, 64):
            if n_out % bn == 0:
                return bn
        return 256 if n_out > 256 else ((n_out + 63) // 64) * 64
    for bn in (256, 160, 128, 96, 64, 32):
        if n_out % bn == 0:
            return bn
    return 256 if n_out > 256 else ((n_out + 31) // 32) * 32


_NUM_SMS = [0]


def num_sms() -> int:
    if _NUM_SMS[0] == 0:
        _NUM_SMS[0] = int(load().svdx_num_sms())
    return _NUM_SMS[0]


_L2_BYTES_PER_CLK = 4500.0


def _tile_cost(M: int, n_out: int, bn_out: int, geglu: bool, sms: int) -> float:
    bn = 2 * bn_out if geglu else bn_out
    ctas = ((M + 127) // 128) * ((n_out + bn_out - 1) // bn_out)
    active = min(ctas, sms)
    mma = 4 * max(bn / 2.0, 32.0 + bn / 4.0)
    l2 = (16384 + 128 * bn) * active / _L2_BYTES_PER_CLK
    waves = (ctas + sms - 1) // sms
    return waves * max(mma, l2)


def choose_block_n(M: int, n_out: int, geglu: bool = False, mn_major: bool = False) -> int:
    sms = num_sms()
    if mn_major:
        best, best_cost = None, None
        m_tiles = (M + 127) // 128
        for bn in (128, 64):
            cost = m_tiles * ((n_out + bn - 1) // bn) * max(bn / 2.0, 32.0 + bn / 4.0)
            if best_cost is None or cost < best_cost - 1e-9:
                best, best_cost = bn, cost
        return best
    cands = [64, 32] if geglu else [160, 128, 96, 64, 32]
    best, best_cost = None, None
    for bn in cands:
        if n_out % bn and n_out > bn:
            continue
        cost = _tile_cost(M, n_out, bn, geglu, sms)
        if best_cost is None or cost < best_cost * 0.98:
            best, best_cost = bn, cost
    if best is None:
        best = pick_block_n(n_out, False)
    return 2 * best if geglu else best


WIDE_TILE = os.environ.get("SVDX_WIDE", "1") != "0"
WIDE_MIN_K = int(os.environ.get("SVDX_WIDE_MIN_K", "960"))


def _wide_tile_ok(M, N, k_total, out, ldo, geglu, a_mn, b_mn, b_mode, split_k, out_dtype, bias, rowbias) -> bool:
    if not WIDE_TILE or geglu or a_mn or b_mn or b_mode != 0 or split_k != 1 or N % 320 or N % 256 == 0 or M < 512 or k_total < WIDE_MIN_K:
        return False
    if out.dtype != bf16 or (out_dtype is not None and out_dtype != OUT_BF16):
        return False
    ld = ldo if ldo is not None else out.stride(0)
    if ld % 8 or out.data_ptr() % 16:
        return False
    if bias is not None and bias.data_ptr() % 16:
        return False
    if rowbias is not None and (rowbias.data_ptr() % 16 or rowbias.stride(0) % 4):
        return False
    return True


_WGRAD_L2_BYTES_PER_CLK = 6500.0


def wgrad_plan(O: int, K: int, M: int):
    sms = num_sms()
    kb = (M + 63) // 64
    m_tiles = (O + 127) // 128
    best = None
    for bn in ((128, 64) if K > 64 else (64,)):
        n_tiles = (K + bn - 1) // bn
        tiles = m_tiles * n_tiles
        splits = {1, max(1, min(kb // 32, sms // max(tiles, 1))), max(1, min(kb // 8, -(-sms // max(tiles, 1))))}
        for split in sorted(splits):
            ctas = tiles * split
            active = min(ctas, sms)
            bytes_kb = 16384 + 128.0 * K / n_tiles
            per = max(4.0 * max(bn / 2.0, 32.0 + bn / 4.0), bytes_kb * active / _WGRAD_L2_BYTES_PER_CLK)
            waves = -(-ctas // sms)
            cost = waves * ((kb / split) * per + bn * 8.0 + 3000.0)
            if best is None or cost < best[0] * 0.97:
                best = (cost, bn, split)
    return best[1], best[2]


def tapgemm(
    a: torch.Tensor,
    b: torch.Tensor,
    out: torch.Tensor,
    *,
    M: int,
    N: int,
    K: int,
    mode: int = A_ROWS,
    taps: Sequence[Sequence[int]] = ((0, 0, 0),),
    rows_per_group: Optional[int] = None,
    groups: int = 1,
    conv_whn: Optional[Sequence[int]] = None,
    lda: Optional[int] = None,
    ldb: Optional[int] = None,
    ldo: Optional[int] = None,
    a_mn: bool = False,
    b_mn: bool = False,
    b_mode: int = 0,
    block_n: Optional[int] = None,
    split_k: int = 1,
    out_dtype: Optional[int] = None,
    geglu: bool = False,
    bias: Optional[torch.Tensor] = None,
    rowbias: Optional[torch.Tensor] = None,
    rowbias_div: int = 1,
    res1: Optional[torch.Tensor] = None,
    res2: Optional[torch.Tensor] = None,
    scales: Optional[torch.Tensor] = None,
    pre: Optional[torch.Tensor] = None,
    gn_sum: Optional[torch.Tensor] = None,
    gn_rows: int = 0,
    gnb: Optional[dict] = None,
    phase: Optional[Sequence[int]] = None,
    act: int = ACT_NONE,
) -> torch.Tensor:
    family = "conv" if (mode == A_CONV2D or len(taps) > 1 or b_mode != 0) else "linear"
    if _fam(family, 2.0 * M * N * K * len(taps)):
        return out
    if SHAPE_LOG is not None:
        SHAPE_LOG.append(dict(M=M, N=N, K=K, taps=len(taps), conv2d=int(mode == A_CONV2D), geglu=int(geglu), a_mn=int(a_mn), b_mode=b_mode,
                              split_k=split_k, block_n=block_n, f32out=int(out.dtype != bf16), bias=int(bias is not None),
                              rowbias=int(rowbias is not None), res=int(res1 is not None) + int(res2 is not None),
                              scales=int(scales is not None), pre=int(pre is not None)))
    d = SvdxTapGemm()
    assert a.dtype == bf16 and b.dtype == bf16
    d.a = a.data_ptr()
    d.lda = lda if lda is not None else _rowmajor(a, "a")
    d.a_mode = mode
    d.a_major_mn = int(a_mn)
    d.rows_per_group = rows_per_group if rows_per_group is not None else M
    d.groups = groups
    if conv_whn is not None:
        d.W, d.H, d.nimg = conv_whn
    d.num_taps = len(taps)
    for i, t in enumerate(taps):
        d.tap_d0[i], d.tap_d1[i], d.tap_d2[i] = int(t[0]), int(t[1]), int(t[2])
    d.b = b.data_ptr()
    d.ldb = ldb if ldb is not None else _rowmajor(b, "b")
    d.b_major_mn = int(b_mn)
    d.b_mode = b_mode
    d.M, d.N, d.K = M, N, K
    n_out = N // 2 if geglu else N
    if block_n is None:
        block_n = choose_block_n(M, n_out, geglu, b_mn)
        if _wide_tile_ok(M, N, K * len(taps), out, ldo, geglu, a_mn, b_mn, b_mode, split_k, out_dtype, bias, rowbias):
            block_n = 320
    d.block_n = block_n
    d.split_k = split_k
    d.out = out.data_ptr()
    d.ldo = ldo if ldo is not None else _rowmajor(out, "out")
    if out_dtype is None:
        out_dtype = OUT_BF16 if out.dtype == bf16 else OUT_F32
    d.out_dtype = out_dtype
    d.geglu = int(geglu)
    if bias is not None:
        assert bias.dtype == torch.float32
        d.bias = bias.data_ptr()
    if rowbias is not None:
        assert rowbias.dtype == torch.float32
        d.rowbias = rowbias.data_ptr()
        d.rowbias_div = rowbias_div
        d.ldrb = _rowmajor(rowbias, "rowbias")
    if res1 is not None:
        assert res1.dtype == bf16
        d.res1 = res1.data_ptr()
        d.ldr1 = _rowmajor(res1, "res1")
    if res2 is not None:
        assert res2.dtype == bf16
        d.res2 = res2.data_ptr()
        d.ldr2 = _rowmajor(res2, "res2")
    if scales is not None:
        assert scales.dtype == torch.float32 and scales.numel() >= 3
        d.scales = scales.data_ptr()
    if pre is not None:
        assert pre.dtype == bf16
        d.pre = pre.data_ptr()
        d.ldpre = _rowmajor(pre, "pre")
    if gn_sum is not None:
        assert gn_sum.dtype == torch.float32 and gn_sum.dim() == 3 and gn_sum.shape[1] == 2 and gn_sum.is_contiguous() and gn_rows > 0
        d.gn_sum = gn_sum.data_ptr()
        d.gn_ld = gn_sum.shape[2]
        d.gn_rows = gn_rows
    if gnb is not None:
        gx, gx2 = gnb["x"], gnb.get("x2")
        assert gx.dtype == bf16 and gnb["sum"].dtype == torch.float32 and gnb["sum"].is_contiguous() and gnb["sum"].shape[-1] == N
        d.gnb_x = gx.data_ptr()
        d.gnb_ldx = _rowmajor(gx, "gnb x")
        if gx2 is not None:
            d.gnb_x2 = gx2.data_ptr()
            d.gnb_ldx2 = _rowmajor(gx2, "gnb x2")
            d.gnb_c1 = gx.shape[-1]
        d.gnb_ab = _ptr(gnb.get("ab"))
        d.gnb_sum = gnb["sum"].data_ptr()
        d.gnb_rows = gnb["rows"]
        d.gnb_silu = int(gnb["silu"])
    if phase is not None:
        d.interleave = 1
        d.phase_h, d.phase_w = int(phase[0]), int(phase[1])
    d.act = int(act)
    check(load().svdx_tapgemm(C.byref(d), _stream()), "svdx_tapgemm")
    return out


_SPLITK_WS: dict = {}


def _splitk_workspace(M: int, N: int, device) -> torch.Tensor:
    key = (M, N, str(device), _stream() if torch.device(device).type == "cuda" else 0)
    ws = _SPLITK_WS.get(key)
    if ws is None:
        ws = torch.zeros(M, N, device=device, dtype=torch.float32)
        _SPLITK_WS[key] = ws
    return ws


def split_plan(out_is_bf16: bool, M: int, N: int, K: int, ntaps: int = 1, geglu=False, a_mn=False, b_mn=False, block_n=None):
    if not (out_is_bf16 and not geglu and not a_mn and not b_mn and block_n is None and N % 8 == 0 and N >= 256):
        return None
    bn = 256 if N % 256 == 0 else (160 if N % 160 == 0 else 0)
    if not bn:
        return None
    kb = ((K + 63) // 64) * ntaps
    tiles = ((M + 127) // 128) * (N // bn)
    split = min(num_sms() // max(tiles, 1), kb // 8)
    if tiles <= num_sms() // 3 and split >= 2:
        return bn, split
    return None


def tapgemm_auto(a, b, out, *, M, N, K, taps=((0, 0, 0),), bias=None, rowbias=None, rowbias_div=1, res1=None, res2=None,
                 scales=None, gn_sum=None, gn_rows=0, **kw):
    kw = dict(kw)
    if kw.get("block_n") is None:
        kw.pop("block_n", None)
    if (M <= 8 and not kw.get("act") and len(taps) == 1 and kw.get("mode", A_ROWS) == A_ROWS and not kw.get("geglu") and not kw.get("a_mn") and not kw.get("b_mn")
            and rowbias is None and res1 is None and res2 is None and scales is None and gn_sum is None and kw.get("groups", 1) == 1
            and K % 8 == 0 and a.stride(-1) == 1 and b.stride(-1) == 1 and out.dtype in (bf16, torch.float32)):
        return gemv(a, b, out, M=M, N=N, K=K, bias=bias, lda=kw.get("lda"), ldw=kw.get("ldb"))
    plan = None if kw.get("act") else split_plan(out.dtype == bf16, M, N, K, len(taps), kw.get("geglu"), kw.get("a_mn"), kw.get("b_mn"),
                                                 kw.get("block_n"))
    if plan is not None:
        assert gn_sum is None, "fused GroupNorm statistics are not available on the split-K path"
        bn, split = plan
        ws = _splitk_workspace(M, N, out.device)
        tapgemm(a, b, ws, M=M, N=N, K=K, taps=taps, block_n=bn, split_k=split, out_dtype=OUT_F32_ATOMIC, **kw)
        if _fam("conv" if (kw.get("mode", A_ROWS) == A_CONV2D or len(taps) > 1) else "linear"):
            return out
        check(load().svdx_splitk_epilogue(ws.data_ptr(), N, out.data_ptr(), _rowmajor(out, "out"), M, N, _ptr(bias), _ptr(rowbias),
                                          rowbias_div, _rowmajor(rowbias, "rowbias") if rowbias is not None else 0,
                                          _ptr(res1), _rowmajor(res1, "res1") if res1 is not None else 0,
                                          _ptr(res2), _rowmajor(res2, "res2") if res2 is not None else 0,
                                          _ptr(scales), _stream()), "svdx_splitk_epilogue")
        return out
    return tapgemm(a, b, out, M=M, N=N, K=K, taps=taps, bias=bias, rowbias=rowbias, rowbias_div=rowbias_div, res1=res1, res2=res2,
                   scales=scales, gn_sum=gn_sum, gn_rows=gn_rows, **kw)


CONV3x3_TAPS = tuple((kw - 1, kh - 1, 0) for kh in range(3) for kw in range(3))


def _attn_desc(q, k, v, o, heads, S, nseq, inner, outer_stride, inner_stride, tok_stride, scale, lse):
    d = SvdxAttn()
    d.q, d.k, d.v, d.o = q.data_ptr(), k.data_ptr(), v.data_ptr(), o.data_ptr()
    d.ldq, d.ldk, d.ldv, d.ldo = _rowmajor(q, "q"), _rowmajor(k, "k"), _rowmajor(v, "v"), _rowmajor(o, "o")
    d.nseq, d.heads, d.S, d.inner = nseq, heads, S, inner
    d.outer_stride, d.inner_stride, d.tok_stride = outer_stride, inner_stride, tok_stride
    d.scale = scale
    d.lse = _ptr(lse)
    return d


def attention_fwd(q, k, v, o, *, heads, S, nseq, inner=1, outer_stride=None, inner_stride=0, tok_stride=1,
                  scale=0.125, lse=None):
    if outer_stride is None:
        outer_stride = S
    if _fam("attention", 4.0 * nseq * heads * S * S * 64):
        return o
    d = _attn_desc(q, k, v, o, heads, S, nseq, inner, outer_stride, inner_stride, tok_stride, scale, lse)
    check(load().svdx_attention_fwd(C.byref(d), _stream()), "svdx_attention_fwd")
    return o


def attention_bwd(q, k, v, o, dout, dq, dk, dv, lse, delta, *, heads, S, nseq, inner=1, outer_stride=None,
                  inner_stride=0, tok_stride=1, scale=0.125):
    if outer_stride is None:
        outer_stride = S
    if _fam("attention", 10.0 * nseq * heads * S * S * 64):
        return
    d = _attn_desc(q, k, v, o, heads, S, nseq, inner, outer_stride, inner_stride, tok_stride, scale, lse)
    d.dout, d.lddo = dout.data_ptr(), _rowmajor(dout, "dout")
    d.dq, d.dk, d.dv = dq.data_ptr(), dk.data_ptr(), dv.data_ptr()
    d.lddq, d.lddk, d.lddv = _rowmajor(dq, "dq"), _rowmajor(dk, "dk"), _rowmajor(dv, "dv")
    d.delta = delta.data_ptr()
    check(load().svdx_attention_bwd(C.byref(d), _stream()), "svdx_attention_bwd")


def attention_hd80_fwd(q, k, v, o, *, heads, S, nseq, scale):
    for t, n in ((q, "q"), (k, "k"), (v, "v"), (o, "o")):
        if t.dtype != bf16 or not t.is_cuda or t.shape[0] < nseq * S:
            raise ValueError(f"attention_hd80_fwd: {n} must be a CUDA bf16 [nseq*S, ld] matrix")
    if _fam("attention", 4.0 * nseq * heads * S * S * 80):
        return o
    check(load().svdx_attention_hd80_fwd(q.data_ptr(), _rowmajor(q, "q"), k.data_ptr(), _rowmajor(k, "k"), v.data_ptr(), _rowmajor(v, "v"),
                                         o.data_ptr(), _rowmajor(o, "o"), nseq, heads, S, float(scale), _stream()), "svdx_attention_hd80_fwd")
    return o


def groupnorm_sums(x, x2, outer, rows, sums=None):
    C1 = x.shape[-1]
    C2 = x2.shape[-1] if x2 is not None else 0
    if sums is None:
        sums = torch.zeros(outer, 2, C1 + C2, device=x.device, dtype=torch.float32)
    if _fam("groupnorm", 0.0, 2.0 * x.shape[0] * (C1 + C2)):
        return sums
    assert sums.dtype == torch.float32 and sums.dim() == 3 and sums.shape[:2] == (outer, 2) and sums.is_contiguous()
    check(load().svdx_groupnorm_sums(x.data_ptr(), _rowmajor(x, "x"), C1, _ptr(x2), _rowmajor(x2, "x2") if x2 is not None else 0, C2,
                                     outer, rows, sums.data_ptr(), sums.shape[2], _stream()), "svdx_groupnorm_sums")
    return sums


def groupnorm_apply_fused(x, x2, outer, rows, eps, csum1, csum2, gamma, beta, silu, y, groups=32, ab=None):
    C1 = x.shape[-1]
    C2 = x2.shape[-1] if x2 is not None else 0
    stats = torch.empty(2, outer * groups, device=x.device, dtype=torch.float32)
    mean, rstd = stats[0], stats[1]
    if _fam("groupnorm", 0.0, 4.0 * x.shape[0] * (C1 + C2)):
        return mean, rstd
    check(load().svdx_groupnorm_apply_fused(x.data_ptr(), _rowmajor(x, "x"), C1, _ptr(x2), _rowmajor(x2, "x2") if x2 is not None else 0, C2,
                                            outer, rows, groups, eps, csum1.data_ptr(), csum1.stride(1),
                                            _ptr(csum2), csum2.stride(1) if csum2 is not None else 0, mean.data_ptr(), rstd.data_ptr(),
                                            gamma.data_ptr(), beta.data_ptr(), int(silu), y.data_ptr(), _rowmajor(y, "y"), _ptr(ab), _stream()),
          "svdx_groupnorm_apply_fused")
    return mean, rstd


def groupnorm_bwd_sums(x, x2, dy, outer, rows, ab, silu, sums=None):
    C1 = x.shape[-1]
    C2 = x2.shape[-1] if x2 is not None else 0
    if sums is None:
        sums = torch.zeros(outer, 2, C1 + C2, device=x.device, dtype=torch.float32)
    if _fam("groupnorm", 0.0, 4.0 * x.shape[0] * (C1 + C2)):
        return sums
    assert sums.dtype == torch.float32 and sums.shape == (outer, 2, C1 + C2) and sums.is_contiguous()
    check(load().svdx_groupnorm_bwd_sums(x.data_ptr(), _rowmajor(x, "x"), C1, _ptr(x2), _rowmajor(x2, "x2") if x2 is not None else 0, C2,
                                         dy.data_ptr(), _rowmajor(dy, "dy"), outer, rows, _ptr(ab), int(silu), sums.data_ptr(), _stream()),
          "svdx_groupnorm_bwd_sums")
    return sums


def groupnorm_bwd_fused(x, x2, dy, outer, rows, mean, rstd, gamma, beta, silu, csum, dx, dx2, dgamma=None, dbeta=None, groups=32, dres=None):
    C1 = x.shape[-1]
    C2 = x2.shape[-1] if x2 is not None else 0
    if _fam("groupnorm", 0.0, 6.0 * x.shape[0] * (C1 + C2)):
        return
    check(load().svdx_groupnorm_bwd_fused(x.data_ptr(), _rowmajor(x, "x"), C1, _ptr(x2), _rowmajor(x2, "x2") if x2 is not None else 0, C2,
                                          dy.data_ptr(), _rowmajor(dy, "dy"), outer, rows, groups, mean.data_ptr(), rstd.data_ptr(),
                                          gamma.data_ptr(), beta.data_ptr(), int(silu), csum.data_ptr(), dx.data_ptr(), _rowmajor(dx, "dx"),
                                          _ptr(dx2), _rowmajor(dx2, "dx2") if dx2 is not None else 0, _ptr(dgamma), _ptr(dbeta),
                                          _ptr(dres), _rowmajor(dres, "dres") if dres is not None else 0, _stream()),
          "svdx_groupnorm_bwd_fused")


def layernorm_fwd(x, gamma, beta, eps, y, addvec=None, add_div=1, xsum=None):
    rows, Cc = x.shape
    mean = torch.empty(rows, device=x.device, dtype=torch.float32)
    rstd = torch.empty_like(mean)
    if _fam("layernorm", 0.0, (6.0 if xsum is not None else 4.0) * rows * Cc):
        return mean, rstd
    check(load().svdx_layernorm_fwd(x.data_ptr(), _rowmajor(x, "x"), rows, Cc, gamma.data_ptr(), beta.data_ptr(), eps,
                                    y.data_ptr(), _rowmajor(y, "y"), mean.data_ptr(), rstd.data_ptr(), _ptr(addvec), add_div,
                                    _ptr(xsum), _rowmajor(xsum, "xsum") if xsum is not None else 0, _stream()), "layernorm_fwd")
    return mean, rstd


def layernorm_bwd(x, dy, gamma, mean, rstd, dx, dres=None, dgamma=None, dbeta=None):
    rows, Cc = x.shape
    if _fam("layernorm", 0.0, (8.0 if dres is not None else 6.0) * rows * Cc):
        return
    check(load().svdx_layernorm_bwd(x.data_ptr(), _rowmajor(x, "x"), dy.data_ptr(), _rowmajor(dy, "dy"), rows, Cc, gamma.data_ptr(),
                                    mean.data_ptr(), rstd.data_ptr(), dx.data_ptr(), _rowmajor(dx, "dx"), _ptr(dres),
                                    _rowmajor(dres, "dres") if dres is not None else 0, _ptr(dgamma), _ptr(dbeta), _stream()),
          "layernorm_bwd")


def prep_weight(src, dst, mode, O, I, taps=1, i_pad=None):
    check(load().svdx_prep_weight(src.data_ptr(), dtype_code(src, "weight"), dst.data_ptr(), mode, O, I, taps,
                                  i_pad if i_pad is not None else I, _stream()), "prep_weight")
    return dst


def cast_f32_bf16(src, dst):
    if _fam("elementwise", 0.0, 6.0 * src.numel()):
        return dst
    check(load().svdx_cast_f32_bf16(src.data_ptr(), dst.data_ptr(), src.numel(), _stream()), "cast_f32_bf16")
    return dst


def cast_bf16_f32(src, dst):
    check(load().svdx_cast_bf16_f32(src.data_ptr(), dst.data_ptr(), src.numel(), _stream()), "cast_bf16_f32")
    return dst


def cast_to_f32(src, dst):
    code = dtype_code(src, "vector")
    if code == 1:
        return cast_bf16_f32(src, dst)
    if code == 2:
        check(load().svdx_cast_f16_f32(src.data_ptr(), dst.data_ptr(), src.numel(), _stream()), "cast_f16_f32")
        return dst
    raise TypeError("cast_to_f32: source is already fp32")


def nchw_to_nhwc(src, dst, N, Cc, H, W, c_pad):
    check(load().svdx_nchw_to_nhwc(src.data_ptr(), dtype_code(src, "NCHW input"), dst.data_ptr(), N, Cc, H, W, c_pad, _stream()), "nchw_to_nhwc")
    return dst


def nhwc_to_nchw(src, dst, N, Cc, H, W):
    check(load().svdx_nhwc_to_nchw(src.data_ptr(), _rowmajor(src, "src"), dst.data_ptr(), dtype_code(dst, "NCHW output"), N, Cc, H, W, _stream()),
          "nhwc_to_nchw")
    return dst


def time_conv_out(x, weight, bias, out, T):
    N, Cc, H, W = out.shape
    if weight.dtype != torch.float32 or not weight.is_contiguous() or weight.numel() != Cc * Cc * 3:
        raise ValueError("time_conv_out: weight must be a contiguous fp32 [C, C, 3(, 1, 1)] tensor")
    if bias is not None and (bias.dtype != torch.float32 or bias.numel() != Cc):
        raise ValueError("time_conv_out: bias must be fp32 [C]")
    if x.dtype != torch.float32 or x.shape[0] != N * H * W:
        raise ValueError("time_conv_out: x must be fp32 [N*H*W, ldx]")
    if _fam("elementwise", 2.0 * 3 * Cc * Cc * out.numel(), 4.0 * x.shape[0] * Cc + out.element_size() * out.numel()):
        return out
    check(load().svdx_time_conv_out(x.data_ptr(), _rowmajor(x, "x"), N, T, Cc, H, W, weight.data_ptr(), _ptr(bias), out.data_ptr(),
                                    dtype_code(out, "time_conv_out output"), _stream()), "svdx_time_conv_out")
    return out


def clip_preprocess(x, gy, gx, affine, out, *, out_size, patch):
    B, Cc, H, W = x.shape
    if Cc != 3 or out.dtype != bf16 or not x.is_cuda or not out.is_cuda:
        raise ValueError("clip_preprocess: x must be a CUDA [B, 3, H, W] image and out a CUDA bf16 matrix")
    if out.shape[0] != B * (1 + (out_size // patch) ** 2):
        raise ValueError("clip_preprocess: out must have B * (1 + P^2) rows")
    gy, gx, affine = [float(v) for v in gy], [float(v) for v in gx], [float(v) for v in affine]
    if len(affine) != 6:
        raise ValueError("clip_preprocess: affine holds 3 scales then 3 shifts")
    strides = (C.c_int64 * 4)(*x.stride())
    fy, fx, fa = (C.c_float * max(1, len(gy)))(*gy), (C.c_float * max(1, len(gx)))(*gx), (C.c_float * 6)(*affine)
    if _fam("elementwise", 0.0, x.element_size() * x.numel() + 2.0 * out.numel()):
        return out
    check(load().svdx_clip_preprocess(x.data_ptr(), dtype_code(x, "image"), strides, B, H, W, fy, len(gy), fx, len(gx), fa, out_size, patch,
                                      out.data_ptr(), _rowmajor(out, "out"), _stream()), "svdx_clip_preprocess")
    return out


def upsample2x(src, dst, N, H, W, Cc):
    check(load().svdx_upsample2x(src.data_ptr(), dst.data_ptr(), N, H, W, Cc, _stream()), "upsample2x")
    return dst


def upsample2x_bwd(dsrc, ddst, N, H, W, Cc):
    check(load().svdx_upsample2x_bwd(dsrc.data_ptr(), ddst.data_ptr(), N, H, W, Cc, _stream()), "upsample2x_bwd")
    return ddst


def space_to_planes(src, dst, N, H, W, Cc):
    check(load().svdx_space_to_planes(src.data_ptr(), dst.data_ptr(), N, H, W, Cc, _stream()), "space_to_planes")
    return dst


def planes_to_space(src, dst, N, H, W, Cc):
    check(load().svdx_planes_to_space(src.data_ptr(), dst.data_ptr(), N, H, W, Cc, _stream()), "planes_to_space")
    return dst


def concat_channels(a, b, dst):
    if _fam("elementwise", 0.0, 4.0 * dst.numel()):
        return dst
    check(load().svdx_concat_channels(a.data_ptr(), a.shape[-1], b.data_ptr(), b.shape[-1], dst.data_ptr(), a.numel() // a.shape[-1],
                                      _stream()), "concat_channels")
    return dst


def split_channels(src, a, b, accumulate_a=False):
    Ca = a.shape[-1]
    Cb = src.shape[-1] - Ca
    if _fam("elementwise", 0.0, 4.0 * src.numel()):
        return
    check(load().svdx_split_channels(src.data_ptr(), a.data_ptr(), Ca, _ptr(b), Cb, src.numel() // src.shape[-1], int(accumulate_a),
                                     _stream()), "split_channels")


def axpby(a, b, y, scales=None):
    if _fam("elementwise", 0.0, 6.0 * a.numel()):
        return y
    check(load().svdx_axpby_bf16(a.data_ptr(), b.data_ptr(), _ptr(scales), y.data_ptr(), a.numel(), _stream()), "axpby_bf16")
    return y


def silu_f32(x, y):
    check(load().svdx_silu_f32(x.data_ptr(), y.data_ptr(), x.numel(), _stream()), "silu_f32")
    return y


def colsum(x, out, accumulate=False):
    rows, cols = x.shape
    if _fam("elementwise", 0.0, 2.0 * rows * cols):
        return out
    check(load().svdx_colsum(x.data_ptr(), _rowmajor(x, "x"), rows, cols, out.data_ptr(), int(accumulate), _stream()), "colsum")
    return out


def geglu_bwd(pre, dout, dpre, bias_grad=None):
    rows, h2 = pre.shape
    if _fam("elementwise", 0.0, 10.0 * rows * (h2 // 2)):
        return dpre
    check(load().svdx_geglu_bwd(pre.data_ptr(), _rowmajor(pre, "pre"), dout.data_ptr(), _rowmajor(dout, "dout"), dpre.data_ptr(),
                                _rowmajor(dpre, "dpre"), rows, h2 // 2, _ptr(bias_grad), _stream()), "geglu_bwd")
    return dpre


def gemv(a, w, out, *, M, N, K, bias=None, lda=None, ldw=None, scale=1.0, accumulate=False):
    if _fam("linear", 2.0 * M * N * K):
        return out
    check(load().svdx_gemv(a.data_ptr(), lda if lda is not None else _rowmajor(a, "a"), w.data_ptr(), ldw if ldw is not None else _rowmajor(w, "w"),
                           M, N, K, _ptr(bias), out.data_ptr(), _rowmajor(out, "out"), OUT_BF16 if out.dtype == bf16 else OUT_F32, float(scale),
                           int(accumulate), _stream()), "svdx_gemv")
    return out


def outer_accum(dy, x, g, scale=None):
    T, O = dy.shape
    K = x.shape[1]
    if _fam("linear", 2.0 * T * O * K):
        return g
    check(load().svdx_outer_accum(dy.data_ptr(), _rowmajor(dy, "dy"), x.data_ptr(), _rowmajor(x, "x"), T, O, K, _ptr(scale), g.data_ptr(),
                                  _rowmajor(g, "g"), _stream()), "svdx_outer_accum")
    return g


def softmax_rows(x, y, scale=1.0):
    rows, cols = x.shape
    if _fam("elementwise", 0.0, 4.0 * rows * cols):
        return y
    check(load().svdx_softmax_rows(x.data_ptr(), _rowmajor(x, "x"), rows, cols, float(scale), y.data_ptr(), _rowmajor(y, "y"), _stream()),
          "svdx_softmax_rows")
    return y


def blend_scales(mix_factor, out3):
    check(load().svdx_blend_scales(mix_factor.data_ptr(), out3.data_ptr(), _stream()), "blend_scales")
    return out3


def adamw(p, g, m, v, lr, beta1, beta2, eps, weight_decay, step, grad_scale=1.0, shadow=None):
    if _fam("adamw", 0.0, (30.0 if shadow is not None else 28.0) * p.numel()):
        return
    check(load().svdx_adamw(p.data_ptr(), g.data_ptr(), m.data_ptr(), v.data_ptr(), p.numel(), lr, beta1, beta2, eps, weight_decay,
                            step, grad_scale, _ptr(shadow), _stream()), "adamw")


def _ema_args(ema, ema_state, n):
    if (ema is None) != (ema_state is None):
        raise ValueError("ema and ema_state go together")
    if ema is not None and (ema.dtype != torch.float32 or ema.numel() != n or ema_state.dtype != torch.float64 or ema_state.numel() < 9):
        raise ValueError("ema: fp32 buffer of the updated slice's length; ema_state: float64[9] (svd_xtend_b200.h)")


def adamw_p2p(p, m, v, peer_grads, peer_shadows, lo, state, grad_scale, tick=True, ema=None, ema_state=None):
    world = len(peer_grads)
    n = p.numel()
    _ema_args(ema, ema_state, n)
    if _fam("adamw", 0.0, (4.0 * world + 28.0 + 2.0 * world + (8.0 if ema is not None else 0.0)) * n):
        return
    ga = (C.c_void_p * world)(*[t if isinstance(t, int) else t.data_ptr() for t in peer_grads])
    sa = (C.c_void_p * world)(*[t if isinstance(t, int) else t.data_ptr() for t in peer_shadows])
    if ema is not None:
        check(load().svdx_adamw_p2p_ema(p.data_ptr(), m.data_ptr(), v.data_ptr(), ga, sa, world, lo, n, state.data_ptr(), float(grad_scale),
                                        int(tick), ema.data_ptr(), ema_state.data_ptr(), _stream()), "svdx_adamw_p2p_ema")
        return
    check(load().svdx_adamw_p2p(p.data_ptr(), m.data_ptr(), v.data_ptr(), ga, sa, world, lo, n, state.data_ptr(), float(grad_scale),
                                int(tick), _stream()), "svdx_adamw_p2p")


def adamw_graph(p, g, m, v, state, grad_scale=1.0, shadow=None, ema=None, ema_state=None):
    _ema_args(ema, ema_state, p.numel())
    if _fam("adamw", 0.0, ((30.0 if shadow is not None else 28.0) + (8.0 if ema is not None else 0.0)) * p.numel()):
        return
    if ema is not None:
        check(load().svdx_adamw_graph_ema(p.data_ptr(), g.data_ptr(), m.data_ptr(), v.data_ptr(), p.numel(), state.data_ptr(), grad_scale,
                                          _ptr(shadow), ema.data_ptr(), ema_state.data_ptr(), _stream()), "svdx_adamw_graph_ema")
        return
    check(load().svdx_adamw_graph(p.data_ptr(), g.data_ptr(), m.data_ptr(), v.data_ptr(), p.numel(), state.data_ptr(), grad_scale,
                                  _ptr(shadow), _stream()), "svdx_adamw_graph")


EMA_CHUNK = 4096


def ema_multi(jobs, block_prefix, njobs, total_blocks, ema_state, nelem):
    if _fam("adamw", 0.0, 12.0 * nelem):
        return
    check(load().svdx_ema_multi(jobs.data_ptr(), block_prefix.data_ptr(), njobs, total_blocks, ema_state.data_ptr(), _stream()),
          "svdx_ema_multi")


A8_BLOCK = 256


def adamw8bit(jobs, block_prefix, njobs, total_blocks, qmap1, qmap2, state, grad_scale=1.0, ema_state=None, nbytes=0.0):
    if qmap1.dtype != torch.float32 or qmap2.dtype != torch.float32 or qmap1.numel() != 256 or qmap2.numel() != 256:
        raise ValueError("adamw8bit: qmap1 / qmap2 are float32[256]")
    if _fam("adamw", 0.0, nbytes):
        return
    if ema_state is not None:
        if ema_state.dtype != torch.float64 or ema_state.numel() < 9:
            raise ValueError("adamw8bit: ema_state is float64[9] (svd_xtend_b200.h)")
        check(load().svdx_adamw8bit_ema(jobs.data_ptr(), block_prefix.data_ptr(), njobs, total_blocks, qmap1.data_ptr(), qmap2.data_ptr(),
                                        state.data_ptr(), float(grad_scale), ema_state.data_ptr(), _stream()), "svdx_adamw8bit_ema")
        return
    check(load().svdx_adamw8bit(jobs.data_ptr(), block_prefix.data_ptr(), njobs, total_blocks, qmap1.data_ptr(), qmap2.data_ptr(),
                                state.data_ptr(), float(grad_scale), _stream()), "svdx_adamw8bit")


def multi_transpose(src_base, jobs, tile_prefix, njobs, total_tiles):
    if _fam("elementwise", 0.0, 4.0 * 64 * 64 * total_tiles):
        return
    check(load().svdx_multi_transpose(src_base.data_ptr(), jobs.data_ptr(), tile_prefix.data_ptr(), njobs, total_tiles, _stream()),
          "svdx_multi_transpose")


def unprep_conv_grad(src, dst, O, I, taps, i_pad):
    check(load().svdx_unprep_conv_grad(src.data_ptr(), dst.data_ptr(), O, I, taps, i_pad, _stream()), "svdx_unprep_conv_grad")
    return dst


def dot_diff(dy, a, b, out):
    check(load().svdx_dot_diff(dy.data_ptr(), a.data_ptr(), b.data_ptr(), dy.numel(), out.data_ptr(), _stream()), "svdx_dot_diff")
    return out


def silu_bwd_f32(x, dy, dx):
    check(load().svdx_silu_bwd_f32(x.data_ptr(), dy.data_ptr(), dx.data_ptr(), x.numel(), _stream()), "svdx_silu_bwd_f32")
    return dx
```

Baseline: 135.5.

## Run fast GEMM epilogues from registers and spend freed smem on deeper pipeline

The fast epilogue variants (FAST, RES, GEGLU, GN, GNB, IL, ACT) now consume the wgmma accumulators straight from registers, using paired-warp staging buffers and named barriers. They no longer park the tile in a shared-memory accumulator buffer behind block-wide barriers. With the accumulator buffer gone, those kernels can use a separate stage count (STAGES_REGS), which allows a deeper TMA pipeline; the generic path keeps the parked layout. MN-major A, and MN-major B with residuals, are routed to the generic path, and the shape log gains full launch metadata. This adds register pressure and a lot of new epilogue code.

After: 151.3 (median of 6 runs). 1.12x the previous value.

```diff
diff --git a/svd_xtend_b200/csrc/tapgemm.cu b/svd_xtend_b200/csrc/tapgemm.cu
--- a/svd_xtend_b200/csrc/tapgemm.cu
+++ b/svd_xtend_b200/csrc/tapgemm.cu
@@ -2,19 +2,22 @@
 
 namespace svdx {
 
-template <int BN, int TA, int TB>
-__device__ __forceinline__ void tile_mainloop(int kb0, int kb1, uint32_t sA, uint32_t sB, uint32_t bar_full, uint32_t bar_empty,
-                                           uint32_t sAcc, int wg, int& stage, uint32_t& phase) {
-  float acc[BN / 2];
+struct Ring {
+  uint32_t sA, sB, bar_full, bar_empty;
+  int stage;
+  uint32_t phase;
+};
+template <int BN, int TA, int TB, int STG>
+__device__ __forceinline__ void tile_mainloop(float (&acc)[BN / 2], int kb0, int kb1, Ring& rg, int wg) {
 #pragma unroll
   for (int i = 0; i < BN / 2; ++i) acc[i] = 0.f;
   const int lane = threadIdx.x & 31;
   const uint32_t astep = TA ? (2048 >> 4) : (32 >> 4), bstep = TB ? (2048 >> 4) : (32 >> 4);
   int prev_stage = -1;
   for (int kb = kb0; kb < kb1; ++kb) {
-    mbar_wait_mma(bar_full + 8 * stage, phase);
-    const uint32_t aaddr = sA + stage * A_STAGE_BYTES + wg * 8192;
-    const uint32_t baddr = sB + stage * B_STAGE_BYTES;
+    mbar_wait_mma(rg.bar_full + 8 * rg.stage, rg.phase);
+    const uint32_t aaddr = rg.sA + rg.stage * A_STAGE_BYTES + wg * 8192;
+    const uint32_t baddr = rg.sB + rg.stage * B_STAGE_BYTES;
     const uint64_t ad0 = make_smem_desc_sw128(aaddr, 8192, 1024);
     const uint64_t bd0 = make_smem_desc_sw128(baddr, 8192, 1024);
     wgmma_fence();
@@ -32,16 +35,22 @@
     reg_fence(acc);
     if (prev_stage >= 0) {
       __syncwarp();
-      if (lane == 0) mbar_arrive(bar_empty + 8 * prev_stage);
-    }
-    prev_stage = stage;
-    if (++stage == STAGES) { stage = 0; phase ^= 1; }
+      if (lane == 0) mbar_arrive(rg.bar_empty + 8 * prev_stage);
+    }
+    prev_stage = rg.stage;
+    if (++rg.stage == STG) { rg.stage = 0; rg.phase ^= 1; }
   }
   wgmma_wait<0>();
   reg_fence(acc);
   __syncwarp();
-  if (lane == 0 && prev_stage >= 0) mbar_arrive(bar_empty + 8 * prev_stage);
-
+  if (lane == 0 && prev_stage >= 0) mbar_arrive(rg.bar_empty + 8 * prev_stage);
+}
+
+template <int BN, int TA, int TB>
+SVDX_DEVINL void tile_parked_bn(int kb0, int kb1, Ring& rg, uint32_t sAcc, int wg) {
+  float acc[BN / 2];
+  tile_mainloop<BN, TA, TB, STAGES_PARKED>(acc, kb0, kb1, rg, wg);
+  const int lane = threadIdx.x & 31;
   const int r0 = wg * 64 + ((threadIdx.x >> 5) & 3) * 16 + (lane >> 2);
   const uint32_t base = sAcc + (uint32_t)(r0 * ACC_LD + 2 * (lane & 3)) * 4u;
 #pragma unroll
@@ -54,25 +63,58 @@
 }
 
 template <int TA, int TB>
-SVDX_DEVINL void tile_mainloop_bn(int bn, int kb0, int kb1, uint32_t sA, uint32_t sB, uint32_t bar_full, uint32_t bar_empty, uint32_t sAcc,
-                                  int wg, int& stage, uint32_t& phase) {
+SVDX_DEVINL void tile_parked(int bn, int kb0, int kb1, Ring& rg, uint32_t sAcc, int wg) {
   switch (bn) {
-    case 32: tile_mainloop<32, TA, TB>(kb0, kb1, sA, sB, bar_full, bar_empty, sAcc, wg, stage, phase); break;
-    case 64: tile_mainloop<64, TA, TB>(kb0, kb1, sA, sB, bar_full, bar_empty, sAcc, wg, stage, phase); break;
-    case 96: tile_mainloop<96, TA, TB>(kb0, kb1, sA, sB, bar_full, bar_empty, sAcc, wg, stage, phase); break;
-    case 128: tile_mainloop<128, TA, TB>(kb0, kb1, sA, sB, bar_full, bar_empty, sAcc, wg, stage, phase); break;
-    default: tile_mainloop<160, TA, TB>(kb0, kb1, sA, sB, bar_full, bar_empty, sAcc, wg, stage, phase); break;
+    case 32: tile_parked_bn<32, TA, TB>(kb0, kb1, rg, sAcc, wg); break;
+    case 64: tile_parked_bn<64, TA, TB>(kb0, kb1, rg, sAcc, wg); break;
+    case 96: tile_parked_bn<96, TA, TB>(kb0, kb1, rg, sAcc, wg); break;
+    case 128: tile_parked_bn<128, TA, TB>(kb0, kb1, rg, sAcc, wg); break;
+    default: tile_parked_bn<160, TA, TB>(kb0, kb1, rg, sAcc, wg); break;
+  }
+}
+
+template <int EPI, int BN, int TB>
+SVDX_DEVINL void tile_regs_bn(const TapGemmKParams& p, int kb0, int kb1, Ring& rg, int wg, PairStage& ps, const EpiTile& t, int lane,
+                              float s_acc, float s_r1, float s_r2) {
+  float acc[BN / 2];
+  tile_mainloop<BN, 0, TB, STAGES_REGS>(acc, kb0, kb1, rg, wg);
+  epilogue_regs<EPI, BN>(p, acc, ps, t, lane, s_acc, s_r1, s_r2);
+}
+
+template <int EPI>
+SVDX_DEVINL void tile_regs(const TapGemmKParams& p, int kb0, int kb1, Ring& rg, int wg, PairStage& ps, const EpiTile& t, int lane,
+                           float s_acc, float s_r1, float s_r2) {
+  if constexpr (EPI == EPI_GEGLU) {
+    if (p.block_n == 64) tile_regs_bn<EPI, 64, 0>(p, kb0, kb1, rg, wg, ps, t, lane, s_acc, s_r1, s_r2);
+    else tile_regs_bn<EPI, 128, 0>(p, kb0, kb1, rg, wg, ps, t, lane, s_acc, s_r1, s_r2);
+  } else {
+    if constexpr (EPI == EPI_FAST) {
+      if (p.b_mn) {
+        if (p.block_n == 64) tile_regs_bn<EPI, 64, 1>(p, kb0, kb1, rg, wg, ps, t, lane, s_acc, s_r1, s_r2);
+        else tile_regs_bn<EPI, 128, 1>(p, kb0, kb1, rg, wg, ps, t, lane, s_acc, s_r1, s_r2);
+        return;
+      }
+    }
+    switch (p.block_n) {
+      case 32: tile_regs_bn<EPI, 32, 0>(p, kb0, kb1, rg, wg, ps, t, lane, s_acc, s_r1, s_r2); break;
+      case 64: tile_regs_bn<EPI, 64, 0>(p, kb0, kb1, rg, wg, ps, t, lane, s_acc, s_r1, s_r2); break;
+      case 96: tile_regs_bn<EPI, 96, 0>(p, kb0, kb1, rg, wg, ps, t, lane, s_acc, s_r1, s_r2); break;
+      case 128: tile_regs_bn<EPI, 128, 0>(p, kb0, kb1, rg, wg, ps, t, lane, s_acc, s_r1, s_r2); break;
+      default: tile_regs_bn<EPI, 160, 0>(p, kb0, kb1, rg, wg, ps, t, lane, s_acc, s_r1, s_r2); break;
+    }
   }
 }
 
 template <int EPI>
 __global__ void __launch_bounds__(NUM_THREADS, 1) tapgemm_kernel(const __grid_constant__ TapGemmKParams p) {
+  constexpr bool PARKED = EPI == EPI_GENERIC;
+  constexpr int STAGES = PARKED ? STAGES_PARKED : STAGES_REGS;
   extern __shared__ uint8_t smem_raw[];
   const uint32_t smem_base = (smem_u32(smem_raw) + 1023u) & ~1023u;
   const uint32_t sA = smem_base;
   const uint32_t sB = smem_base + STAGES * A_STAGE_BYTES;
   const uint32_t sAcc = sB + STAGES * B_STAGE_BYTES;
-  const uint32_t sEpi = sAcc + ACC_BYTES;
+  const uint32_t sEpi = sAcc + (PARKED ? ACC_BYTES : 0);
   const uint32_t sBar = sEpi + NUM_EPI_WARPS * EPI_STAGE_BYTES;
   const uint32_t bar_full = sBar;
   const uint32_t bar_empty = sBar + 8 * STAGES;
@@ -279,10 +321,9 @@
     }
   } else {
     const int wg = warp >> 2;
-    const int q = warp & 3;
-    const int half = warp >> 2;
-    int stage = 0;
-    uint32_t phase = 0;
+    const int q = PARKED ? (warp & 3) : (warp >> 1);
+    const int half = PARKED ? (warp >> 2) : (warp & 1);
+    Ring rg{sA, sB, bar_full, bar_empty, 0, 0u};
     float s_acc = 1.f, s_r1 = 1.f, s_r2 = 1.f;
     if (p.scales) { s_acc = p.scales[0]; s_r1 = p.scales[1]; s_r2 = p.scales[2]; }
     const int n_out_total = p.geglu ? p.N / 2 : p.N;
@@ -290,6 +331,7 @@
     EpiStage st;
     st.base = sEpi + warp * EPI_STAGE_BYTES;
     st.off = 0;
+    PairStage ps{sEpi + q * 2 * EPI_STAGE_BYTES, 2 + q, half, 0u};
     const uint32_t t_base = sAcc + (uint32_t)((q * 32 + lane) * ACC_LD) * 4u;
     for (int tile = blockIdx.x; tile < total_tiles; tile += gridDim.x) {
       const int nt = tile % p.n_tiles;
@@ -319,19 +361,21 @@
       }
       if constexpr (EPI == EPI_RES || EPI == EPI_RES_GN || EPI == EPI_FAST_GNB)
         prefetch_epilogue_operands(p, EPI, m0, valid_rows, n0, bn_out, n_out_total, lane, half);
-      named_bar_sync(1, 32 * NUM_EPI_WARPS);
-      if (p.a_mn && p.b_mn) tile_mainloop_bn<1, 1>(p.block_n, kb0, kb1, sA, sB, bar_full, bar_empty, sAcc, wg, stage, phase);
-      else if (p.a_mn) tile_mainloop_bn<1, 0>(p.block_n, kb0, kb1, sA, sB, bar_full, bar_empty, sAcc, wg, stage, phase);
-      else if (p.b_mn) tile_mainloop_bn<0, 1>(p.block_n, kb0, kb1, sA, sB, bar_full, bar_empty, sAcc, wg, stage, phase);
-      else tile_mainloop_bn<0, 0>(p.block_n, kb0, kb1, sA, sB, bar_full, bar_empty, sAcc, wg, stage, phase);
-      named_bar_sync(1, 32 * NUM_EPI_WARPS);
-      if constexpr (EPI == EPI_FAST || EPI == EPI_FAST_GN) epilogue_fast<EPI == EPI_FAST_GN>(p, t_base, m, row_ok, n0, half, 0, bn_out, n_out_total, st.base, st.row0, st.grp, lane, m0, valid_rows);
-      else if constexpr (EPI == EPI_FAST_IL || EPI == EPI_FAST_IL_GN) epilogue_fast<EPI == EPI_FAST_IL_GN, true>(p, t_base, m, row_ok, n0, half, 0, bn_out, n_out_total, st.base, st.row0, st.grp, lane, m0, valid_rows);
-      else if constexpr (EPI == EPI_FAST_ACT) epilogue_fast<false, false, true>(p, t_base, m, row_ok, n0, half, 0, bn_out, n_out_total, st.base, st.row0, st.grp, lane, m0, valid_rows);
-      else if constexpr (EPI == EPI_RES || EPI == EPI_RES_GN) epilogue_res<EPI == EPI_RES_GN>(p, t_base, m, row_ok, n0, half, 0, bn_out, n_out_total, s_acc, s_r1, s_r2, st.base, st.off, st.row0, st.grp, lane, m0, valid_rows);
-      else if constexpr (EPI == EPI_GEGLU) epilogue_geglu(p, t_base, n0, half, bn_out, st.base, st.row0, st.grp, lane);
-      else if constexpr (EPI == EPI_FAST_GNB) epilogue_fast_gnb(p, t_base, m, row_ok, n0, half, 0, bn_out, n_out_total, st.base, st.row0, st.grp, lane, m0, valid_rows);
-      else epilogue_tile(p, t_base, m, row_ok, n0, half, bn_out, n_out_total, s_acc, s_r1, s_r2, st, lane);
+      if constexpr (PARKED) {
+        named_bar_sync(1, 32 * NUM_EPI_WARPS);
+        if (p.a_mn && p.b_mn) tile_parked<1, 1>(p.block_n, kb0, kb1, rg, sAcc, wg);
+        else if (p.a_mn) tile_parked<1, 0>(p.block_n, kb0, kb1, rg, sAcc, wg);
+        else if (p.b_mn) tile_parked<0, 1>(p.block_n, kb0, kb1, rg, sAcc, wg);
+        else tile_parked<0, 0>(p.block_n, kb0, kb1, rg, sAcc, wg);
+        named_bar_sync(1, 32 * NUM_EPI_WARPS);
+        epilogue_tile(p, t_base, m, row_ok, n0, half, bn_out, n_out_total, s_acc, s_r1, s_r2, st, lane);
+      } else {
+        EpiTile et;
+        et.n0 = n0; et.n_out_total = n_out_total; et.row0 = st.row0; et.grp = st.grp; et.valid_rows = valid_rows; et.m0 = m0;
+#pragma unroll
+        for (int h = 0; h < 2; ++h) tile_row(p, mt, q * 32 + half * 16 + (lane >> 2) + 8 * h, et.m[h], et.ok[h]);
+        tile_regs<EPI>(p, kb0, kb1, rg, wg, ps, et, lane, s_acc, s_r1, s_r2);
+      }
     }
     if (lane == 0) bulk_wait<0>();
   }
@@ -524,8 +568,9 @@
     p.epi_mode = EPI_GENERIC;
     const bool vec_ok = (reinterpret_cast<uintptr_t>(d->bias) & 15) == 0
                         && (!d->rowbias || ((reinterpret_cast<uintptr_t>(d->rowbias) & 15) == 0 && d->ldrb % 4 == 0));
-    if (p.tma_store && !f32 && n_out % 32 == 0 && vec_ok && !p.probe && use != 2)
-      p.epi_mode = d->geglu ? EPI_GEGLU : (d->res1 || d->res2 || d->scales) ? EPI_RES : EPI_FAST;
+    const bool has_res = d->res1 || d->res2 || d->scales;
+    if (p.tma_store && !f32 && n_out % 32 == 0 && vec_ok && !d->a_major_mn && !(d->b_major_mn && has_res) && !p.probe && use != 2)
+      p.epi_mode = d->geglu ? EPI_GEGLU : has_res ? EPI_RES : EPI_FAST;
   }
   if (p.split_k > 1 && (p.bias || p.rowbias || p.res1 || p.res2 || p.geglu)) return svdx_fail(SVDX_E_BADARG, "tapgemm: split_k with epilogue operands");
   if (p.gnb_sum) {
@@ -566,6 +611,8 @@
     p.act = d->act;
     p.epi_mode = EPI_FAST_ACT;
   }
+  if (d->b_major_mn && p.epi_mode != EPI_GENERIC && (p.epi_mode != EPI_FAST || p.gn_sum))
+    return svdx_fail(SVDX_E_BADARG, "tapgemm: MN-major B takes the plain epilogue only (no gn_sum / gnb sums / act)");
   if (wide320 && p.epi_mode != EPI_FAST && p.epi_mode != EPI_RES && p.epi_mode != EPI_FAST_GNB && p.epi_mode != EPI_FAST_IL && p.epi_mode != EPI_FAST_ACT)
     return svdx_fail(SVDX_E_BADARG, "tapgemm: block_n 320 needs a bf16 output through the TMA-store epilogues (N % 320 == 0, aligned rows)");
   if (p.gn_sum) {
@@ -581,6 +628,17 @@
   if (d->pre && ((d->ldpre % 8) || (reinterpret_cast<uintptr_t>(d->pre) & 15))) return svdx_fail(SVDX_E_BADARG, "tapgemm: pre alignment");
 
   return SVDX_OK;
+}
+
+static constexpr int kernel_smem(int epi) { return epi == EPI_GENERIC ? smem_bytes(STAGES_PARKED, true) : smem_bytes(STAGES_REGS, false); }
+
+template <int EPI>
+static cudaError_t set_smem() {
+  return cudaFuncSetAttribute(tapgemm_kernel<EPI>, cudaFuncAttributeMaxDynamicSharedMemorySize, kernel_smem(EPI));
+}
+template <int EPI>
+static void launch(int grid, cudaStream_t stream, const TapGemmKParams& p) {
+  tapgemm_kernel<EPI><<<grid, NUM_THREADS, kernel_smem(EPI), stream>>>(p);
 }
 
 extern "C" int svdx_tapgemm(const SvdxTapGemm* d, void* stream_v) {
@@ -591,32 +649,32 @@
   static bool attr_done[SVDX_MAX_DEVICES] = {false};
   const int slot = svdx_device_slot();
   if (!attr_done[slot]) {
-    cudaError_t e = cudaFuncSetAttribute(tapgemm_kernel<EPI_GENERIC>, cudaFuncAttributeMaxDynamicSharedMemorySize, SMEM_BYTES);
-    if (e == cudaSuccess) e = cudaFuncSetAttribute(tapgemm_kernel<EPI_FAST>, cudaFuncAttributeMaxDynamicSharedMemorySize, SMEM_BYTES);
-    if (e == cudaSuccess) e = cudaFuncSetAttribute(tapgemm_kernel<EPI_GEGLU>, cudaFuncAttributeMaxDynamicSharedMemorySize, SMEM_BYTES);
-    if (e == cudaSuccess) e = cudaFuncSetAttribute(tapgemm_kernel<EPI_RES>, cudaFuncAttributeMaxDynamicSharedMemorySize, SMEM_BYTES);
-    if (e == cudaSuccess) e = cudaFuncSetAttribute(tapgemm_kernel<EPI_FAST_GN>, cudaFuncAttributeMaxDynamicSharedMemorySize, SMEM_BYTES);
-    if (e == cudaSuccess) e = cudaFuncSetAttribute(tapgemm_kernel<EPI_RES_GN>, cudaFuncAttributeMaxDynamicSharedMemorySize, SMEM_BYTES);
-    if (e == cudaSuccess) e = cudaFuncSetAttribute(tapgemm_kernel<EPI_FAST_GNB>, cudaFuncAttributeMaxDynamicSharedMemorySize, SMEM_BYTES);
-    if (e == cudaSuccess) e = cudaFuncSetAttribute(tapgemm_kernel<EPI_FAST_IL>, cudaFuncAttributeMaxDynamicSharedMemorySize, SMEM_BYTES);
-    if (e == cudaSuccess) e = cudaFuncSetAttribute(tapgemm_kernel<EPI_FAST_IL_GN>, cudaFuncAttributeMaxDynamicSharedMemorySize, SMEM_BYTES);
-    if (e == cudaSuccess) e = cudaFuncSetAttribute(tapgemm_kernel<EPI_FAST_ACT>, cudaFuncAttributeMaxDynamicSharedMemorySize, SMEM_BYTES);
+    cudaError_t e = set_smem<EPI_GENERIC>();
+    if (e == cudaSuccess) e = set_smem<EPI_FAST>();
+    if (e == cudaSuccess) e = set_smem<EPI_GEGLU>();
+    if (e == cudaSuccess) e = set_smem<EPI_RES>();
+    if (e == cudaSuccess) e = set_smem<EPI_FAST_GN>();
+    if (e == cudaSuccess) e = set_smem<EPI_RES_GN>();
+    if (e == cudaSuccess) e = set_smem<EPI_FAST_GNB>();
+    if (e == cudaSuccess) e = set_smem<EPI_FAST_IL>();
+    if (e == cudaSuccess) e = set_smem<EPI_FAST_IL_GN>();
+    if (e == cudaSuccess) e = set_smem<EPI_FAST_ACT>();
     if (e != cudaSuccess) return svdx_fail_cuda(e, "tapgemm: set smem attribute");
     attr_done[slot] = true;
   }
   const int total_tiles = p.m_tiles * p.n_tiles * p.split_k;
   int grid = svdx_num_sms();
   if (grid > total_tiles) grid = total_tiles;
-  if (p.epi_mode == EPI_FAST_ACT) tapgemm_kernel<EPI_FAST_ACT><<<grid, NUM_THREADS, SMEM_BYTES, stream>>>(p);
-  else if (p.epi_mode == EPI_FAST_IL && p.gn_sum) tapgemm_kernel<EPI_FAST_IL_GN><<<grid, NUM_THREADS, SMEM_BYTES, stream>>>(p);
-  else if (p.epi_mode == EPI_FAST_IL) tapgemm_kernel<EPI_FAST_IL><<<grid, NUM_THREADS, SMEM_BYTES, stream>>>(p);
-  else if (p.epi_mode == EPI_FAST_GNB) tapgemm_kernel<EPI_FAST_GNB><<<grid, NUM_THREADS, SMEM_BYTES, stream>>>(p);
-  else if (p.epi_mode == EPI_FAST && p.gn_sum) tapgemm_kernel<EPI_FAST_GN><<<grid, NUM_THREADS, SMEM_BYTES, stream>>>(p);
-  else if (p.epi_mode == EPI_RES && p.gn_sum) tapgemm_kernel<EPI_RES_GN><<<grid, NUM_THREADS, SMEM_BYTES, stream>>>(p);
-  else if (p.epi_mode == EPI_FAST) tapgemm_kernel<EPI_FAST><<<grid, NUM_THREADS, SMEM_BYTES, stream>>>(p);
-  else if (p.epi_mode == EPI_GEGLU) tapgemm_kernel<EPI_GEGLU><<<grid, NUM_THREADS, SMEM_BYTES, stream>>>(p);
-  else if (p.epi_mode == EPI_RES) tapgemm_kernel<EPI_RES><<<grid, NUM_THREADS, SMEM_BYTES, stream>>>(p);
-  else tapgemm_kernel<EPI_GENERIC><<<grid, NUM_THREADS, SMEM_BYTES, stream>>>(p);
+  if (p.epi_mode == EPI_FAST_ACT) launch<EPI_FAST_ACT>(grid, stream, p);
+  else if (p.epi_mode == EPI_FAST_IL && p.gn_sum) launch<EPI_FAST_IL_GN>(grid, stream, p);
+  else if (p.epi_mode == EPI_FAST_IL) launch<EPI_FAST_IL>(grid, stream, p);
+  else if (p.epi_mode == EPI_FAST_GNB) launch<EPI_FAST_GNB>(grid, stream, p);
+  else if (p.epi_mode == EPI_FAST && p.gn_sum) launch<EPI_FAST_GN>(grid, stream, p);
+  else if (p.epi_mode == EPI_RES && p.gn_sum) launch<EPI_RES_GN>(grid, stream, p);
+  else if (p.epi_mode == EPI_FAST) launch<EPI_FAST>(grid, stream, p);
+  else if (p.epi_mode == EPI_GEGLU) launch<EPI_GEGLU>(grid, stream, p);
+  else if (p.epi_mode == EPI_RES) launch<EPI_RES>(grid, stream, p);
+  else launch<EPI_GENERIC>(grid, stream, p);
   cudaError_t e = cudaGetLastError();
   if (e != cudaSuccess) return svdx_fail_cuda(e, "tapgemm: launch");
   return SVDX_OK;
diff --git a/svd_xtend_b200/csrc/tapgemm_common.cuh b/svd_xtend_b200/csrc/tapgemm_common.cuh
--- a/svd_xtend_b200/csrc/tapgemm_common.cuh
+++ b/svd_xtend_b200/csrc/tapgemm_common.cuh
@@ -7,7 +7,6 @@
 
 constexpr int BLOCK_M = 128;
 constexpr int BLOCK_K = 64;
-constexpr int STAGES = 3;
 constexpr int MAX_BN = 160;
 constexpr int A_STAGE_BYTES = BLOCK_M * BLOCK_K * 2;
 constexpr int B_STAGE_BYTES = MAX_BN * BLOCK_K * 2;
@@ -17,8 +16,14 @@
 constexpr int ACC_LD = MAX_BN + 4;
 constexpr int ACC_BYTES = BLOCK_M * ACC_LD * 4;
 constexpr int EPI_STAGE_BYTES = 4096;
-constexpr int SMEM_BYTES = 1024 + STAGES * (A_STAGE_BYTES + B_STAGE_BYTES) + ACC_BYTES + NUM_EPI_WARPS * EPI_STAGE_BYTES + 256;
-static_assert(SMEM_BYTES <= 227 * 1024, "tapgemm shared memory exceeds the 227 KB a block may use");
+constexpr int STAGES_PARKED = 3;
+constexpr int STAGES_REGS = 5;
+constexpr int smem_bytes(int stages, bool parked) {
+  return 1024 + stages * (A_STAGE_BYTES + B_STAGE_BYTES) + (parked ? ACC_BYTES : 0) + NUM_EPI_WARPS * EPI_STAGE_BYTES + 256;
+}
+static_assert(smem_bytes(STAGES_PARKED, true) <= 227 * 1024, "tapgemm shared memory exceeds the 227 KB a block may use");
+static_assert(smem_bytes(STAGES_REGS, false) <= 227 * 1024, "tapgemm shared memory exceeds the 227 KB a block may use");
+static_assert(16 * STAGES_REGS <= 256, "ring barriers must fit their 256-byte region");
 static_assert((ACC_BYTES % 1024) == 0 && (B_STAGE_BYTES % 1024) == 0, "staging buffers must stay 1024-byte aligned");
 
 struct __align__(64) TapGemmKParams {
@@ -192,13 +197,14 @@
 constexpr int EPI_FAST_IL = 7, EPI_FAST_IL_GN = 8;
 constexpr int EPI_FAST_ACT = 9;
 
-SVDX_DEVINL void act32(float (&f)[32], int act) {
+template <int N>
+SVDX_DEVINL void act_n(float (&f)[N], int act) {
   if (act == SVDX_ACT_GELU) {
 #pragma unroll
-    for (int i = 0; i < 32; ++i) f[i] = gelu_erf_f(f[i]);
+    for (int i = 0; i < N; ++i) f[i] = gelu_erf_f(f[i]);
   } else {
 #pragma unroll
-    for (int i = 0; i < 32; ++i) f[i] = __fdividef(f[i], 1.0f + __expf(-1.702f * f[i]));
+    for (int i = 0; i < N; ++i) f[i] = __fdividef(f[i], 1.0f + __expf(-1.702f * f[i]));
   }
 }
 
@@ -225,29 +231,6 @@
     asm volatile("ld.shared.v4.b32 {%0, %1, %2, %3}, [%4];" : "=r"(v.x), "=r"(v.y), "=r"(v.z), "=r"(v.w) : "r"(row + ((j ^ sw) << 4)));
     dst[j] = v;
   }
-}
-
-SVDX_DEVINL void add_vec32(float (&f)[32], const float* __restrict__ src) {
-  const float4* bp = reinterpret_cast<const float4*>(src);
-#pragma unroll
-  for (int k = 0; k < 8; ++k) {
-    const float4 b4 = __ldg(bp + k);
-    f[4 * k] += b4.x; f[4 * k + 1] += b4.y; f[4 * k + 2] += b4.z; f[4 * k + 3] += b4.w;
-  }
-}
-SVDX_DEVINL void axpy_bf16x32(float (&f)[32], float s, const uint4 (&r)[4]) {
-#pragma unroll
-  for (int k = 0; k < 4; ++k) {
-    const float2 a = unpack_bf16x2(r[k].x), b = unpack_bf16x2(r[k].y), c = unpack_bf16x2(r[k].z), d = unpack_bf16x2(r[k].w);
-    f[8 * k] += s * a.x; f[8 * k + 1] += s * a.y; f[8 * k + 2] += s * b.x; f[8 * k + 3] += s * b.y;
-    f[8 * k + 4] += s * c.x; f[8 * k + 5] += s * c.y; f[8 * k + 6] += s * d.x; f[8 * k + 7] += s * d.y;
-  }
-}
-SVDX_DEVINL void stage_row_bf16(uint32_t row, int sw, const float (&f)[32]) {
-#pragma unroll
-  for (int j = 0; j < 4; ++j)
-    st_shared_v4(row + ((j ^ sw) << 4), pack_bf16x2(f[8 * j], f[8 * j + 1]), pack_bf16x2(f[8 * j + 2], f[8 * j + 3]),
-                 pack_bf16x2(f[8 * j + 4], f[8 * j + 5]), pack_bf16x2(f[8 * j + 6], f[8 * j + 7]));
 }
 
 SVDX_DEVINL void prefetch_rows_l2(const bf16* base, long long ld, long long m0, int valid_rows, int col0, int ncols, int lane, int half) {
@@ -272,50 +255,7 @@
   }
 }
 
-template <bool GN, bool IL = false, bool ACT = false>
-SVDX_DEVINL void epilogue_fast(const TapGemmKParams& p, uint32_t t_base, long long m, bool row_ok, int n0, int half, int c_lo, int c_hi,
-                               int n_out_total, uint32_t sbase, int row0, int grp, int lane, long long m0, int valid_rows) {
-  const float* bias = p.bias;
-  const float* rb = (p.rowbias && row_ok) ? p.rowbias + (m / p.rowbias_div) * p.ldrb : nullptr;
-  const uint32_t rowX = sbase + lane * 64, rowY = rowX + 2048;
-  const int sw = (lane >> 1) & 3;
-#pragma unroll 1
-  for (int c = c_lo + half * 32; c < c_hi; c += 128) {
-    const int colA = n0 + c;
-    if (colA >= n_out_total) break;
-    const int colB = colA + 64;
-    const bool hasB = (c + 64 < c_hi) && (colB < n_out_total);
-    uint32_t va[32], vb[32];
-    acc_ld32(t_base, c, va);
-    if (hasB) acc_ld32(t_base, c + 64, vb);
-    float fa[32], fb[32];
-#pragma unroll
-    for (int i = 0; i < 32; ++i) { fa[i] = __uint_as_float(va[i]); fb[i] = __uint_as_float(vb[i]); }
-    if (bias) { add_vec32(fa, bias + colA); if (hasB) add_vec32(fb, bias + colB); }
-    if (rb) { add_vec32(fa, rb + colA); if (hasB) add_vec32(fb, rb + colB); }
-    if constexpr (ACT) { act32(fa, p.act); if (hasB) act32(fb, p.act); }
-    if (lane == 0) bulk_wait_read<0>();
-    __syncwarp();
-    stage_row_bf16(rowX, sw, fa);
-    if (hasB) stage_row_bf16(rowY, sw, fb);
-    fence_proxy_async_smem();
-    __syncwarp();
-    if (lane == 0) {
-      store_chunk<IL>(p, sbase, colA, row0, grp);
-      if (hasB) store_chunk<IL>(p, sbase + 2048, colB, row0, grp);
-      bulk_commit();
-    }
-    if constexpr (IL) {
-      il_store_next_row(p, sbase, colA, row0, lane);
-      if (hasB) il_store_next_row(p, sbase + 2048, colB, row0, lane);
-    }
-    if constexpr (GN) {
-      gn_chunk_sums(p, sbase, lane, colA, n_out_total, m0, valid_rows);
-      if (hasB) gn_chunk_sums(p, sbase + 2048, lane, colB, n_out_total, m0, valid_rows);
-    }
-  }
-}
-
+template <int ROWS = 32>
 SVDX_DEVINL void gnb_chunk_sums(const TapGemmKParams& p, uint32_t buf_dy, uint32_t buf_x, int lane, int col0, int n_out_total, long long m0,
                                 int valid_rows) {
   const int pr = lane & 15, h = lane >> 4;
@@ -334,9 +274,9 @@
       B = *reinterpret_cast<const float2*>(p.gnb_ab + (2 * slab + 1) * p.N + col);
     }
     float s0 = 0.f, s1 = 0.f, x0 = 0.f, x1 = 0.f;
-    if (r == 0 && seg_end == 32) {
-#pragma unroll
-      for (int b = 0; b < 2; ++b) {
+    if (r == 0 && seg_end == ROWS) {
+#pragma unroll
+      for (int b = 0; b < ROWS / 16; ++b) {
         uint32_t wd[8], wx[8];
 #pragma unroll
         for (int i = 0; i < 8; ++i) {
@@ -389,161 +329,178 @@
   }
 }
 
-SVDX_DEVINL void epilogue_fast_gnb(const TapGemmKParams& p, uint32_t t_base, long long m, bool row_ok, int n0, int half, int c_lo, int c_hi,
-                                   int n_out_total, uint32_t sbase, int row0, int grp, int lane, long long m0, int valid_rows) {
+struct PairStage {
+  uint32_t slots;
+  int bar;
+  int sub;
+  uint32_t round;
+};
+struct EpiTile {
+  int n0, n_out_total, row0, grp, valid_rows;
+  long long m0;
+  long long m[2];
+  bool ok[2];
+};
+
+SVDX_DEVINL uint32_t sw64(int r, int j) { return (uint32_t)(r * 64 + ((j ^ ((r >> 1) & 3)) << 4)); }
+SVDX_DEVINL uint32_t frag_row_addr(uint32_t base16, int lane, int x) {
+  const int mi = lane >> 3;
+  return base16 + sw64(8 * (mi & 1) + (lane & 7), 2 * x + (mi >> 1));
+}
+SVDX_DEVINL void stmatrix_x4(uint32_t addr, uint32_t a, uint32_t b, uint32_t c, uint32_t d) {
+  asm volatile("stmatrix.sync.aligned.m8n8.x4.shared.b16 [%0], {%1, %2, %3, %4};" ::"r"(addr), "r"(a), "r"(b), "r"(c), "r"(d) : "memory");
+}
+SVDX_DEVINL void ldmatrix_x4(uint32_t addr, uint32_t& a, uint32_t& b, uint32_t& c, uint32_t& d) {
+  asm volatile("ldmatrix.sync.aligned.m8n8.x4.shared.b16 {%0, %1, %2, %3}, [%4];" : "=r"(a), "=r"(b), "=r"(c), "=r"(d) : "r"(addr) : "memory");
+}
+SVDX_DEVINL void stage_frag16(uint32_t base16, int lane, const float (&f)[16]) {
+#pragma unroll
+  for (int x = 0; x < 2; ++x)
+    stmatrix_x4(frag_row_addr(base16, lane, x), pack_bf16x2(f[8 * x], f[8 * x + 1]), pack_bf16x2(f[8 * x + 2], f[8 * x + 3]),
+                pack_bf16x2(f[8 * x + 4], f[8 * x + 5]), pack_bf16x2(f[8 * x + 6], f[8 * x + 7]));
+}
+SVDX_DEVINL void load_rows16(const bf16* base, long long ld, int nrows, int lane, uint4 (&v)[2]) {
+#pragma unroll
+  for (int j = 0; j < 2; ++j) {
+    const int rr = (lane >> 2) + 8 * j;
+    v[j] = rr < nrows ? *reinterpret_cast<const uint4*>(base + (long long)rr * ld + (lane & 3) * 8) : make_uint4(0u, 0u, 0u, 0u);
+  }
+}
+SVDX_DEVINL void stage_rows16(uint32_t base16, int lane, const uint4 (&v)[2]) {
+#pragma unroll
+  for (int j = 0; j < 2; ++j) st_shared_v4(base16 + sw64((lane >> 2) + 8 * j, lane & 3), v[j].x, v[j].y, v[j].z, v[j].w);
+}
+
+template <int EPI, int BN>
+SVDX_DEVINL void epilogue_regs(const TapGemmKParams& p, const float (&acc)[BN / 2], PairStage& ps, const EpiTile& t, int lane, float s_acc,
+                               float s_r1, float s_r2) {
+  constexpr bool GEGLU = EPI == EPI_GEGLU;
+  constexpr bool RES = EPI == EPI_RES || EPI == EPI_RES_GN;
+  constexpr bool GN = EPI == EPI_FAST_GN || EPI == EPI_RES_GN || EPI == EPI_FAST_IL_GN;
+  constexpr bool IL = EPI == EPI_FAST_IL || EPI == EPI_FAST_IL_GN;
+  constexpr bool GNB = EPI == EPI_FAST_GNB;
+  constexpr int BN_OUT = GEGLU ? BN / 2 : BN;
+  const int cq = 2 * (lane & 3);
+  const bool issuer = ps.sub == 0 && lane == 0;
+  const bool save_pre = GEGLU && p.pre != nullptr;
+  const int vr = t.valid_rows - 16 * ps.sub;
+  const long long mw = t.m0 + 16 * ps.sub;
   const float* bias = p.bias;
-  const float* rb = (p.rowbias && row_ok) ? p.rowbias + (m / p.rowbias_div) * p.ldrb : nullptr;
-  const uint32_t rowX = sbase + lane * 64;
-  const int sw = (lane >> 1) & 3;
-  const int prow = lane >> 2, ppc = lane & 3;
-#pragma unroll 1
-  for (int c = c_lo + half * 32; c < c_hi; c += 64) {
-    const int col0 = n0 + c;
-    if (col0 >= n_out_total) break;
-    const bool src1 = col0 < p.gnb_c1;
-    const long long xld = src1 ? p.gnb_ldx : p.gnb_ldx2;
-    const bf16* xs = (src1 ? p.gnb_x + col0 : p.gnb_x2 + (col0 - p.gnb_c1)) + m0 * xld + ppc * 8;
-    uint4 xa[4];
-#pragma unroll
-    for (int j = 0; j < 4; ++j) {
-      const int rr = prow + 8 * j;
-      xa[j] = (rr < valid_rows) ? *reinterpret_cast<const uint4*>(xs + (long long)rr * xld) : make_uint4(0u, 0u, 0u, 0u);
-    }
-    uint32_t v[32];
-    acc_ld32(t_base, c, v);
-    float f[32];
-#pragma unroll
-    for (int i = 0; i < 32; ++i) f[i] = __uint_as_float(v[i]);
-    if (bias) add_vec32(f, bias + col0);
-    if (rb) add_vec32(f, rb + col0);
-    if (lane == 0) bulk_wait_read<0>();
-    __syncwarp();
-    stage_row_bf16(rowX, sw, f);
-#pragma unroll
-    for (int j = 0; j < 4; ++j) {
-      const int rr = prow + 8 * j;
-      st_shared_v4(sbase + 2048 + rr * 64 + ((ppc ^ ((rr >> 1) & 3)) << 4), xa[j].x, xa[j].y, xa[j].z, xa[j].w);
-    }
+  const float* rb[2] = {nullptr, nullptr};
+  const bf16* r2[2] = {nullptr, nullptr};
+#pragma unroll
+  for (int h = 0; h < 2; ++h) {
+    if (!GEGLU && p.rowbias) rb[h] = p.rowbias + (t.ok[h] ? t.m[h] / p.rowbias_div : 0) * p.ldrb;
+    if (RES && p.res2) r2[h] = p.res2 + (t.ok[h] ? t.m[h] : 0) * p.ldr2;
+  }
+#pragma unroll
+  for (int ch = 0; ch < BN_OUT / 32; ++ch) {
+    const int col0 = t.n0 + 32 * ch;
+    if (col0 >= t.n_out_total) break;
+    const uint32_t slot = ps.slots + 2048u * (GNB ? 2 * (ps.round & 1) : save_pre ? 2 : (ps.round & 3));
+    const uint32_t mine = slot + 1024u * ps.sub;
+    uint4 xa[2];
+    if constexpr (RES) {
+      if (p.res1) load_rows16(p.res1 + mw * p.ldr1 + col0, p.ldr1, vr, lane, xa);
+    }
+    if constexpr (GNB) {
+      const bool src1 = col0 < p.gnb_c1;
+      const long long xld = src1 ? p.gnb_ldx : p.gnb_ldx2;
+      load_rows16((src1 ? p.gnb_x + col0 : p.gnb_x2 + (col0 - p.gnb_c1)) + mw * xld, xld, vr, lane, xa);
+    }
+    uint32_t a2[8];
+    if constexpr (RES) {
+      if (p.res2) {
+#pragma unroll
+        for (int k = 0; k < 8; ++k) a2[k] = *reinterpret_cast<const uint32_t*>(r2[k & 1] + col0 + 8 * (k >> 1) + cq);
+      }
+    }
+    float f[16], g[16];
+#pragma unroll
+    for (int i = 0; i < 16; ++i) {
+      f[i] = acc[16 * ch + i];
+      if constexpr (GEGLU) g[i] = acc[BN_OUT / 2 + 16 * ch + i];
+    }
+    if (bias) {
+#pragma unroll
+      for (int j = 0; j < 4; ++j) {
+        const float2 b = __ldg(reinterpret_cast<const float2*>(bias + col0 + 8 * j + cq));
+        f[4 * j] += b.x; f[4 * j + 1] += b.y; f[4 * j + 2] += b.x; f[4 * j + 3] += b.y;
+        if constexpr (GEGLU) {
+          const float2 bg = __ldg(reinterpret_cast<const float2*>(bias + p.N / 2 + col0 + 8 * j + cq));
+          g[4 * j] += bg.x; g[4 * j + 1] += bg.y; g[4 * j + 2] += bg.x; g[4 * j + 3] += bg.y;
+        }
+      }
+    }
+    if (!GEGLU && p.rowbias) {
+#pragma unroll
+      for (int k = 0; k < 8; ++k) {
+        const float2 b = __ldg(reinterpret_cast<const float2*>(rb[k & 1] + col0 + 8 * (k >> 1) + cq));
+        f[2 * k] += b.x; f[2 * k + 1] += b.y;
+      }
+    }
+    if constexpr (EPI == EPI_FAST_ACT) act_n(f, p.act);
+    if constexpr (RES) {
+      if (p.scales) {
+#pragma unroll
+        for (int i = 0; i < 16; ++i) f[i] = __fmul_rn(f[i], s_acc);
+      }
+      if (p.res1) {
+        uint32_t a1[8];
+        stage_rows16(mine, lane, xa);
+        __syncwarp();
+        ldmatrix_x4(frag_row_addr(mine, lane, 0), a1[0], a1[1], a1[2], a1[3]);
+        ldmatrix_x4(frag_row_addr(mine, lane, 1), a1[4], a1[5], a1[6], a1[7]);
+        __syncwarp();
+#pragma unroll
+        for (int k = 0; k < 8; ++k) {
+          const float2 a = unpack_bf16x2(a1[k]);
+          f[2 * k] = __fmaf_rn(s_r1, a.x, f[2 * k]); f[2 * k + 1] = __fmaf_rn(s_r1, a.y, f[2 * k + 1]);
+        }
+      }
+      if (p.res2) {
+#pragma unroll
+        for (int k = 0; k < 8; ++k) {
+          const float2 a = unpack_bf16x2(a2[k]);
+          f[2 * k] = __fmaf_rn(s_r2, a.x, f[2 * k]); f[2 * k + 1] = __fmaf_rn(s_r2, a.y, f[2 * k + 1]);
+        }
+      }
+    }
+    if constexpr (GEGLU) {
+      if (save_pre) {
+        stage_frag16(ps.slots + 1024u * ps.sub, lane, f);
+        stage_frag16(ps.slots + 2048u + 1024u * ps.sub, lane, g);
+        fence_proxy_async_smem();
+        if (issuer) bulk_wait_read<0>();
+        named_bar_sync(ps.bar, 64);
+        if (issuer) {
+          tma_store_3d(&p.tmpre, ps.slots, col0, t.row0, t.grp);
+          tma_store_3d(&p.tmpre, ps.slots + 2048u, p.N / 2 + col0, t.row0, t.grp);
+          bulk_commit();
+        }
+      }
+#pragma unroll
+      for (int i = 0; i < 16; ++i) {
+        const float fv = __bfloat162float(__float2bfloat16(f[i]));
+        const float gv = __bfloat162float(__float2bfloat16(g[i]));
+        f[i] = fv * gelu_erf_f(gv);
+      }
+    }
+    stage_frag16(mine, lane, f);
+    if constexpr (GNB) stage_rows16(mine + 2048u, lane, xa);
     fence_proxy_async_smem();
-    __syncwarp();
-    if (lane == 0) { tma_store_3d(&p.tmo, sbase, col0, row0, grp); bulk_commit(); }
-    gnb_chunk_sums(p, sbase, sbase + 2048, lane, col0, n_out_total, m0, valid_rows);
-    __syncwarp();
-  }
-}
-
-template <bool GN>
-SVDX_DEVINL void epilogue_res(const TapGemmKParams& p, uint32_t t_base, long long m, bool row_ok, int n0, int half, int c_lo, int c_hi,
-                              int n_out_total, float s_acc, float s_r1, float s_r2, uint32_t sbase, uint32_t& off, int row0, int grp, int lane,
-                              long long m0, int valid_rows) {
-  const float* bias = p.bias;
-  const float* rb = (p.rowbias && row_ok) ? p.rowbias + (m / p.rowbias_div) * p.ldrb : nullptr;
-  const bf16* r1 = p.res1 ? p.res1 + m0 * p.ldr1 : nullptr;
-  const bf16* r2 = (p.res2 && row_ok) ? p.res2 + m * p.ldr2 : nullptr;
-  const bool scaled = p.scales != nullptr;
-  const uint32_t row = sbase + lane * 64;
-  const int sw = (lane >> 1) & 3;
-  const int prow = lane >> 2, ppc = lane & 3;
-#pragma unroll 1
-  for (int c = c_lo + half * 32; c < c_hi; c += 64) {
-    const int col0 = n0 + c;
-    if (col0 >= n_out_total) break;
-    uint4 a1[4], a2[4];
-    if (r1) {
-#pragma unroll
-      for (int j = 0; j < 4; ++j) {
-        const int rr = prow + 8 * j;
-        a1[j] = (rr < valid_rows) ? *reinterpret_cast<const uint4*>(r1 + (long long)rr * p.ldr1 + col0 + ppc * 8) : make_uint4(0u, 0u, 0u, 0u);
-      }
-    }
-    if (r2) {
-      const uint4* q = reinterpret_cast<const uint4*>(r2 + col0);
-#pragma unroll
-      for (int k = 0; k < 4; ++k) a2[k] = q[k];
-    }
-    uint32_t v[32];
-    acc_ld32(t_base, c, v);
-    float f[32];
-#pragma unroll
-    for (int i = 0; i < 32; ++i) f[i] = __uint_as_float(v[i]);
-    if (bias) add_vec32(f, bias + col0);
-    if (rb) add_vec32(f, rb + col0);
-    if (scaled) {
-#pragma unroll
-      for (int i = 0; i < 32; ++i) f[i] *= s_acc;
-    }
-    if (lane == 0) bulk_wait_read<1>();
-    __syncwarp();
-    if (r1) {
-#pragma unroll
-      for (int j = 0; j < 4; ++j) {
-        const int rr = prow + 8 * j;
-        st_shared_v4(sbase + off + rr * 64 + ((ppc ^ ((rr >> 1) & 3)) << 4), a1[j].x, a1[j].y, a1[j].z, a1[j].w);
-      }
-      __syncwarp();
-#pragma unroll
-      for (int k = 0; k < 4; ++k)
-        asm volatile("ld.shared.v4.b32 {%0, %1, %2, %3}, [%4];" : "=r"(a1[k].x), "=r"(a1[k].y), "=r"(a1[k].z), "=r"(a1[k].w) : "r"(row + off + ((k ^ sw) << 4)));
-      axpy_bf16x32(f, s_r1, a1);
-    }
-    if (r2) axpy_bf16x32(f, s_r2, a2);
-    stage_row_bf16(row + off, sw, f);
-    fence_proxy_async_smem();
-    __syncwarp();
-    if (lane == 0) { tma_store_3d(&p.tmo, sbase + off, col0, row0, grp); bulk_commit(); }
-    if constexpr (GN) gn_chunk_sums(p, sbase + off, lane, col0, n_out_total, m0, valid_rows);
-    off ^= 2048;
-  }
-}
-
-SVDX_DEVINL void epilogue_geglu(const TapGemmKParams& p, uint32_t t_base, int n0, int half, int bn_out, uint32_t sbase, int row0,
-                                int grp, int lane) {
-  const float* bias = p.bias;
-  const bool save_pre = p.pre != nullptr;
-  const int nh = p.N / 2;
-  const uint32_t rowX = sbase + lane * 64, rowY = rowX + 2048;
-  const int sw = (lane >> 1) & 3;
-  uint32_t off = 0;
-#pragma unroll 1
-  for (int c = half * 32; c < bn_out; c += 64) {
-    const int col0 = n0 + c;
-    uint32_t v[32], gte[32];
-    acc_ld32(t_base, c, v);
-    acc_ld32(t_base, bn_out + c, gte);
-    float f[32], g[32];
-#pragma unroll
-    for (int i = 0; i < 32; ++i) { f[i] = __uint_as_float(v[i]); g[i] = __uint_as_float(gte[i]); }
-    if (bias) { add_vec32(f, bias + col0); add_vec32(g, bias + nh + col0); }
-    if (save_pre) {
-      if (lane == 0) bulk_wait_read<0>();
-      __syncwarp();
-      stage_row_bf16(rowX, sw, f);
-      stage_row_bf16(rowY, sw, g);
-      fence_proxy_async_smem();
-      __syncwarp();
-      if (lane == 0) {
-        tma_store_3d(&p.tmpre, sbase, col0, row0, grp);
-        tma_store_3d(&p.tmpre, sbase + 2048, nh + col0, row0, grp);
-        bulk_commit();
-      }
-    }
-#pragma unroll
-    for (int i = 0; i < 32; ++i) {
-      const float fv = __bfloat162float(__float2bfloat16(f[i]));
-      const float gv = __bfloat162float(__float2bfloat16(g[i]));
-      f[i] = fv * gelu_erf_f(gv);
-    }
-    if (save_pre) {
-      if (lane == 0) bulk_wait_read<0>();
-    } else {
-      if (lane == 0) bulk_wait_read<1>();
-    }
-    __syncwarp();
-    stage_row_bf16(save_pre ? rowX : rowX + off, sw, f);
-    fence_proxy_async_smem();
-    __syncwarp();
-    if (lane == 0) { tma_store_3d(&p.tmo, save_pre ? sbase : sbase + off, col0, row0, grp); bulk_commit(); }
-    off ^= 2048;
+    if (issuer) {
+      if (GNB || save_pre) bulk_wait_read<0>();
+      else bulk_wait_read<2>();
+    }
+    named_bar_sync(ps.bar, 64);
+    if (issuer) { store_chunk<IL>(p, slot, col0, t.row0, t.grp); bulk_commit(); }
+    if constexpr (IL) {
+      if ((ps.round & 1) == (uint32_t)ps.sub) il_store_next_row(p, slot, col0, t.row0, lane);
+    }
+    if constexpr (GN) gn_chunk_sums(p, mine, lane, col0, t.n_out_total, mw, max(0, min(16, vr)));
+    if constexpr (GNB) gnb_chunk_sums<16>(p, mine, mine + 2048u, lane, col0, t.n_out_total, mw, max(0, min(16, vr)));
+    ++ps.round;
   }
 }
 
diff --git a/svd_xtend_b200/raw.py b/svd_xtend_b200/raw.py
--- a/svd_xtend_b200/raw.py
+++ b/svd_xtend_b200/raw.py
@@ -48,6 +48,10 @@
 
 def _ptr(t: Optional[torch.Tensor]) -> Optional[int]:
     return None if t is None else t.data_ptr()
+
+
+def _layout(t: torch.Tensor) -> dict:
+    return dict(shape=list(t.shape), stride=list(t.stride()), dtype=str(t.dtype).replace("torch.", ""))
 
 
 def _rowmajor(t: torch.Tensor, name: str) -> int:
@@ -199,7 +203,19 @@
         SHAPE_LOG.append(dict(M=M, N=N, K=K, taps=len(taps), conv2d=int(mode == A_CONV2D), geglu=int(geglu), a_mn=int(a_mn), b_mode=b_mode,
                               split_k=split_k, block_n=block_n, f32out=int(out.dtype != bf16), bias=int(bias is not None),
                               rowbias=int(rowbias is not None), res=int(res1 is not None) + int(res2 is not None),
-                              scales=int(scales is not None), pre=int(pre is not None)))
+                              scales=int(scales is not None), pre=int(pre is not None),
+                              launch=dict(M=M, N=N, K=K, mode=mode, taps=[[int(v) for v in t] for t in taps], rows_per_group=rows_per_group,
+                                          groups=groups, conv_whn=None if conv_whn is None else [int(v) for v in conv_whn], lda=lda, ldb=ldb,
+                                          ldo=ldo, a_mn=bool(a_mn), b_mn=bool(b_mn), b_mode=b_mode, block_n=block_n, split_k=split_k,
+                                          out_dtype=out_dtype, geglu=bool(geglu), rowbias_div=rowbias_div, gn_rows=gn_rows,
+                                          phase=None if phase is None else [int(v) for v in phase], act=int(act),
+                                          gnb=None if gnb is None else dict(rows=int(gnb["rows"]), silu=bool(gnb["silu"])),
+                                          tensors={k: _layout(t) for k, t in (
+                                              ("a", a), ("b", b), ("out", out), ("bias", bias), ("rowbias", rowbias), ("res1", res1),
+                                              ("res2", res2), ("scales", scales), ("pre", pre), ("gn_sum", gn_sum),
+                                              ("gnb_x", None if gnb is None else gnb["x"]), ("gnb_x2", None if gnb is None else gnb.get("x2")),
+                                              ("gnb_ab", None if gnb is None else gnb.get("ab")), ("gnb_sum", None if gnb is None else gnb["sum"]))
+                                              if t is not None})))
     d = SvdxTapGemm()
     assert a.dtype == bf16 and b.dtype == bf16
     d.a = a.data_ptr()
```
